# hmakelin/gisnav

Measured on AMD Instinct MI355X. Metric: matched frame-pairs/sec + PnP poses/sec, 640x480 cam-vs-tile, higher is better.
Workload: dtype f32-accurate FFN / out-projection / match-head GEMMs (each f32 operand split into 2 fp16 terms = 22 significant bits, 3 fp16 MFMA partial products, f32 accumulate; fp16-range guard active); attention INPUT projections (q, k, v: 18 of 66 launches) on 2 partial products -- the fp16 high term of the ac

## Files before the change

### gisnav_amd/csrc/gn_api.hip

```cpp
#include "gn_common.h"

#include <cstdio>
#include <cstring>
#include <cmath>
#include <cctype>
#include <algorithm>
#include <tuple>

using namespace gn;

namespace {

thread_local std::string g_err;

struct Linear { float* w = nullptr; float* b = nullptr; int out = 0, in = 0; uint16_t* wp = nullptr; float acc_scale = 1.f;
                uint16_t* wf = nullptr; int frag_order = -1;
                uint16_t* wf2 = nullptr;
                uint16_t* wfn = nullptr; };

struct Block {
  Linear proj_in;
  Linear proj_out;
  Linear ffn0;
  float* ln_g = nullptr; float* ln_b = nullptr;
// ... 3 lines not shown

enum Stage { ST_PREP = 0, ST_PROJ, ST_ATTN, ST_FFN, ST_HEAD, ST_GATHER, ST_PNP, ST_COUNT };

struct Call {
  int B = 0, kpt_format = 0, stride_q = 0, stride_r = 0;
  const float *desc_q = nullptr, *kpt_q = nullptr, *desc_r = nullptr, *kpt_r = nullptr; const int32_t *n_q = nullptr, *n_r = nullptr;
  const uint8_t* dem = nullptr; int H = 0, W = 0;
  double *R = nullptr, *t = nullptr; int32_t *n_match = nullptr, *n_inliers = nullptr; uint8_t* ok = nullptr; int64_t* idx = nullptr; float* score = nullptr;
  double *cov = nullptr, *sigma_hat = nullptr; uint8_t* cov_ok = nullptr; double sigma_px = 0.0;
  const double* K9 = nullptr; int min_matches = 0;
  int kw = 0, in_dim = 0; size_t km = 0;
  Call() = default;
  Call(int feature, int npad, int B_, int kpt_format_, const float* desc_q_, const float* kpt_q_, const int32_t* n_q_, int stride_q_,
       const float* desc_r_, const float* kpt_r_, const int32_t* n_r_, int stride_r_)
      : B(B_), kpt_format(kpt_format_), stride_q(stride_q_), stride_r(stride_r_), desc_q(desc_q_), kpt_q(kpt_q_), desc_r(desc_r_), kpt_r(kpt_r_),
        n_q(n_q_), n_r(n_r_), kw((kpt_format_ & 0xff) == GN_KPT_LAF ? 6 : (kpt_format_ & 0xff) == GN_KPT_RECORD ? kRecordFloats : 4),
        in_dim(feature == GN_FEATURE_SIFT ? kInDim : kDim), km((size_t)npad) {}
};

template <typename F, typename... C> void pair_arrays(const Call& h, F&& f, C&... c) {
  f((size_t)h.stride_q * h.in_dim * 4, false, c.desc_q...); f((size_t)h.stride_r * h.in_dim * 4, false, c.desc_r...);
  f((size_t)h.stride_q * h.kw * 4, false, c.kpt_q...); f((size_t)h.stride_r * h.kw * 4, false, c.kpt_r...);
  f((size_t)4, false, c.n_q...); f((size_t)4, false, c.n_r...); f((size_t)h.H * h.W, false, c.dem...);
  f((size_t)72, true, c.R...); f((size_t)24, true, c.t...); f((size_t)4, true, c.n_match...); f((size_t)4, true, c.n_inliers...); f((size_t)1, true, c.ok...);
  f(h.km * 16, true, c.idx...); f(h.km * 4, true, c.score...);
  f((size_t)288, true, c.cov...); f((size_t)8, true, c.sigma_hat...); f((size_t)1, true, c.cov_ok...);
}
template <typename T> T* byte_offset(T* p, size_t bytes) { return reinterpret_cast<T*>(reinterpret_cast<uintptr_t>(p) + bytes); }

Call slice(const Call& v, size_t b0, int n) {
  Call o = v;
  o.B = n;
  pair_arrays(o, [&](size_t bytes, bool, auto*& p) { if (p) p = byte_offset(p, b0 * bytes); }, o);
  return o;
}

template <typename... T> struct Restore {
  std::tuple<T&...> ref; std::tuple<T...> val;
  explicit Restore(T&... r) : ref(r...), val(r...) {}
  ~Restore() { ref = val; }
  Restore(const Restore&) = delete;
  Restore& operator=(const Restore&) = delete;
};

}

struct gn_ctx {
  int device = 0, max_batch = 0, npad = 0, precision = 0;
  int x_planes_only = 1;
  int qkv_stamps = 0;
  int qkv_fused = 1;
  int sp_split = 1;
  long long sp_split_trips = 0;
  int sp_stop = 0;
  int sp_ts_layer = 0;
  long long* sp_ts = nullptr;
  void* sp_allocs_dbg = nullptr;
  bool sp_enc_hm16 = false, sp_enc_fp16 = false;
  int head_fused = 1;
  int head_stamps = 0;
  int pnp_stamps = 0;
  int ffn_compose = 1;
  int ffn_fold = 1;
  int ffn_fused = 3;
  unsigned int* ovf_base = nullptr; unsigned int* ovf = nullptr; unsigned int* ovf_host = nullptr;
  int dbg_trip_group = 0;
  bool in_group = false;
  int ovf_groups_last = 1;
  int guard = 1;
  long long guard_trips = 0;
  int certify = 0;
  float cert_eps = 4.0e-3f;
  int cert_eps_src = 0;
  float cert_eps_f32 = 1.0e-4f;
  float* max0b = nullptr; float* rpart_c = nullptr; int32_t* uncert = nullptr; int32_t* uncert_alt = nullptr; int32_t* uncert_host = nullptr;
  bool cert_inner = false;
  void* cert_stage = nullptr; size_t cert_stage_bytes = 0;
  struct CertPending {
    bool active = false; hipEvent_t ev = nullptr; int32_t* flags = nullptr;
    int npad_run = 0, level = 0;
    Call call; double K9[9] = {0};
  } cert_pend[2];
  int cert_slot = 0;
  long long cert_calls = 0, cert_pairs = 0, cert_flag_margin = 0, cert_flag_range = 0, cert_rerun = 0, cert_f32_marginal = 0;
  int attn_f16 = 0;
  int ladder = 0; float cert_eps_mid = -1.f, cert_mid_measured = -1.f;
  long long mid_rerun = 0, mid_certified = 0, mid_passed = 0;
  float *colbest = nullptr, *col2 = nullptr;
  bool cal_cols = false;
  int precision_api = 0;
  int feature = 0;
  float size_q[2] = {0.f, 0.f}, size_r[2] = {0.f, 0.f};
  int npad_run = 0;
  int n_layers = kMaxLayers;
  float threshold = 0.5f;
  std::string err;
  Linear input_proj;
  float* wr = nullptr;
  Block self_blk[kMaxLayers], cross_blk[kMaxLayers];
  Linear final_proj[kMaxLayers], matchability[kMaxLayers];
  std::map<std::string, bool> loaded;
  std::vector<std::string> required;
  float *desc = nullptr, *cos_t = nullptr, *sin_t = nullptr, *extent = nullptr;
  int32_t* nvalid = nullptr;
  float *x = nullptr, *qkv = nullptr, *ctx = nullptr, *msg = nullptr, *h = nullptr, *md = nullptr, *ls = nullptr;
  uint16_t *desc_p = nullptr, *x_p = nullptr, *ctx_p = nullptr, *msg_p = nullptr, *h_p = nullptr, *md_p = nullptr;
  size_t Tmax = 0;
  int planes_mode = 0;
  float* sim = nullptr;
  uint16_t *qkb = nullptr, *vtb = nullptr;
  float* attn_part = nullptr; unsigned int* attn_tickets = nullptr;
  int attn_split = 1;
  int attn_variant = 4;
  int stop_after = 0;
  int launch_count = 0;
  int no_planes = 0;
  int dbg_planes = 0;
  uint16_t* dbg_wp = nullptr; size_t dbg_wp_n = 0;
  int dbg_out = 0;
  uint16_t* dbg_yp = nullptr; size_t dbg_yp_n = 0;
  int dbg_vt_skip = 0;
  int dbg_reuse = 0;
  uint16_t* dbg_ap = nullptr; size_t dbg_ap_n = 0;
  int gemm_variant = -1;
  float *rowmax = nullptr, *rowlog = nullptr, *colmax = nullptr, *collog = nullptr, *max0 = nullptr;
  int32_t *m0 = nullptr, *m1 = nullptr;
  float *cpart_m = nullptr, *cpart_s = nullptr;
  int32_t* cpart_i = nullptr;
  float* rot4 = nullptr;
  float *rpart_a = nullptr, *rpart_b = nullptr;
  unsigned int* tickets = nullptr;
  int64_t* e_idx = nullptr; float* e_score = nullptr; float* e_mkp = nullptr; float* e_obj = nullptr;
  int defer_join = 0, sub_last_B = 0, sub_last_np = 0;
  int sub_serial = 0;
  int cu_mask_mode = 0;
  int use_lists = 1;
  int ncu = 256;
  int fused_proj_status = -1;
  bool fused_proj_pending = true;
  int fused_proj_off = 0;
  int qkv_in_tail = 1;
  int skinny = 1;
  int auto_level = 3; float cert_eps_lvl[2] = {-1.f, -1.f}; long long auto_pairs = 0, auto_wide = 0, auto_narrow = 0, auto_calls_lvl[2] = {0, 0}, auto_switches = 0;
  int ffn_products = 3;
  int qkv_products = 2;
  unsigned long long* tile_feedback = nullptr;
  int* lists = nullptr; long long lists_stride = 0;
  int n_sub = 1; hipStream_t sub_s[8] = {}; hipEvent_t ev_fork = nullptr; hipEvent_t ev_join[8] = {}; bool sub_pending[8] = {};
  int overlap = 0; unsigned long long calls = 0;
  hipStream_t s_pnp = nullptr; hipEvent_t ev_gather[2][8] = {}, ev_pnp[2][8] = {}; bool pnp_pending[2][8] = {}, pnp_recorded[2][8] = {};
  hipEvent_t ev_head[8] = {};
  float* o_mkp[2] = {nullptr, nullptr}; float* o_obj[2] = {nullptr, nullptr}; int32_t* o_nmatch[2] = {nullptr, nullptr};
  int prep_fused = 1;
  int sift_h = 0, sift_w = 0; std::vector<void*> sift_allocs; SiftPyramid sift_py; float* sift_tmp = nullptr;
  float* sift_dk = nullptr; std::vector<std::vector<float>> sift_kernels; std::vector<int> sift_koff;
  int4* sift_cand = nullptr; int* sift_counts = nullptr; SiftKeypoint* sift_kp = nullptr;
  int sift_max_cand = 0, sift_max_kp = 0, sift_raw_cap = 0, sift_batch = 0; long long sift_kp_stride = 0;
  std::vector<int32_t> sift_totals;
  struct SpConv { float* wf = nullptr; float* b = nullptr; int cout = 0, cin = 0, taps = 0, cout_pad = 0; bool have_w = false, have_b = false;
                  uint16_t* wfh = nullptr; float acc_scale = 1.f; };
  SpConv sp[12];
  std::vector<void*> sp_allocs; int sp_h = 0, sp_w = 0, sp_chunk = 0, sp_cap = 0, sp_max = 0;
  float *sp_x = nullptr, *sp_y = nullptr, *sp_z = nullptr, *sp_maps[6] = {};
  int *sp_cand = nullptr, *sp_counts = nullptr, *sp_index = nullptr;
  float* vo_norm2 = nullptr; int32_t* vo_nn_idx = nullptr; float* vo_nn_dist = nullptr; uint8_t* vo_good = nullptr;
  uint8_t* mask_ws = nullptr;
  float* pts_ws = nullptr;
  gn::HypResult* hyp_ws = nullptr;
  std::vector<void*> allocs;
  std::vector<void*> ws_allocs;
  bool timing = false;
  hipEvent_t ev[2 * 128];
  int ev_stage[128]; int n_ev = 0; bool ev_ready = false;
  float stage_ms[ST_COUNT] = {0};
  bool ktiming = false;
  std::vector<hipEvent_t> kev;
  std::vector<double> kflops;
  std::vector<double> kbytes;
  std::vector<int> kclass;
  std::vector<const char*> kname;
  size_t kused = 0;
};

namespace {

#define GN_HIP(call)                                                                              \
  do {                                                                                            \
    hipError_t e_ = (call);                                                                       \
    if (e_ != hipSuccess) {                                                                       \
      char buf_[512];                                                                             \
      snprintf(buf_, sizeof buf_, "%s failed: %s (%s:%d)", #call, hipGetErrorString(e_), __FILE__, __LINE__); \
      if (ctx) ctx->err = buf_;                                                                   \
      g_err = buf_;                                                                               \
      return GN_ERR_HIP;                                                                          \
    }                                                                                             \
  } while (0)

int fail(gn_ctx* ctx, int code, const std::string& msg) {
  if (ctx) ctx->err = msg;
  g_err = msg;
  return code;
}

template <typename T>
int dalloc(gn_ctx* ctx, T** p, size_t count) {
  void* q = nullptr;
  GN_HIP(hipMalloc(&q, count * sizeof(T)));
  GN_HIP(hipMemset(q, 0, count * sizeof(T)));
  ctx->allocs.push_back(q);
  *p = reinterpret_cast<T*>(q);
  return GN_OK;
}

template <typename T_>
int ws_alloc(gn_ctx* ctx, T_** p, size_t count) {
  void* q = nullptr;
  GN_HIP(hipMalloc(&q, count * sizeof(T_)));
  GN_HIP(hipMemset(q, 0, count * sizeof(T_)));
  ctx->ws_allocs.push_back(q);
  *p = reinterpret_cast<T_*>(q);
  return GN_OK;
}
int ensure_sim(gn_ctx* ctx) {
  if (ctx->sim) return GN_OK;
  return ws_alloc(ctx, &ctx->sim, (size_t)ctx->max_batch * ctx->npad * ctx->npad);
}

std::string canonical(const std::string& k) {
  for (const char* kind : {"self_attn.", "cross_attn."}) {
    const size_t L = strlen(kind);
    if (k.compare(0, L, kind) == 0) {
      const size_t dot = k.find('.', L);
      if (dot == std::string::npos) return k;
      return "transformers." + k.substr(L, dot - L) + "." + std::string(kind) + k.substr(dot + 1);
    }
  }
  return k;
}

struct StageTimer {
  gn_ctx* c; hipStream_t s; int st;
  StageTimer(gn_ctx* c_, hipStream_t s_, int st_) : c(c_), s(s_), st(st_) {
    if (c->timing && c->n_ev < 128) { hipEventRecord(c->ev[2 * c->n_ev], s); }
  }
  ~StageTimer() {
    if (c->timing && c->n_ev < 128) { hipEventRecord(c->ev[2 * c->n_ev + 1], s); c->ev_stage[c->n_ev] = st; ++c->n_ev; }
  }
};

bool planes_of(gn_ctx* c, const float* p, uint16_t** planes) {
  struct { const float* f; uint16_t* q; size_t cols; } tab[] = {
    {c->desc, c->desc_p, (size_t)kInDim}, {c->x, c->x_p, (size_t)kDim}, {c->ctx, c->ctx_p, (size_t)kDim},
    {c->msg, c->msg_p, (size_t)kDim}, {c->h, c->h_p, (size_t)2 * kDim}, {c->md, c->md_p, (size_t)kDim}};
  for (auto& e : tab) {
    if (e.f && p >= e.f && p < e.f + c->Tmax * e.cols && (size_t)(p - e.f) % e.cols == 0) {
      *planes = e.q + 2 * (p - e.f);
      return true;
    }
  }
  return false;
}

template <typename F> bool timed_launch(gn_ctx* c, hipStream_t s, int kclass, double flops, double bytes, const char* name, F&& launch) {
  ++c->launch_count;
  if (c->stop_after && c->launch_count > c->stop_after) return false;
  const bool rec = c->ktiming && c->kused < c->kflops.size();
  if (rec) hipEventRecord(c->kev[2 * c->kused], s);
  launch();
  if (rec) {
    hipEventRecord(c->kev[2 * c->kused + 1], s);
    c->kflops[c->kused] = flops; c->kbytes[c->kused] = bytes; c->kclass[c->kused] = kclass; c->kname[c->kused] = name ? name : gn::g_last_kernel;
    ++c->kused;
  }
  return true;
}

void timed_gemm(gn_ctx* c, int epi, const GemmArgs& g_in, int batch, hipStream_t s) {
  if (c->gemm_variant >= 0) gn::g_gemm_variant = c->gemm_variant;
  GemmArgs g = g_in;
  if (c->no_planes) g.Wp = nullptr;
  bool p2 = false;
  if (c->planes_mode) {
    uint16_t* q = nullptr;
    p2 = planes_of(c, g.A, &q);
    if (p2) {
      g.Ap = q;
      if (g.A2) { uint16_t* q2 = nullptr; p2 = planes_of(c, g.A2, &q2) && g.lda2 == g.lda; g.A2p = q2; }
    }
    if (p2 && !g.Wp) {
      uint16_t* qw = nullptr;
      p2 = planes_of(c, g.W, &qw);
      g.Wp = qw; g.acc_scale = 1.f;
    }
    if (p2) g.ovf = c->guard ? c->ovf : nullptr;
    if (p2) {
      uint16_t* qy = nullptr;
      if (g.Y == c->x) { planes_of(c, g.Y, &qy); g.Yp = qy; g.ldyp = g.ldy; if (g.drop_f32) g.Y = nullptr; }
      else if (g.Y == c->msg || g.Y == c->md) { planes_of(c, g.Y, &qy); g.Yp = qy; g.ldyp = g.ldy; g.Y = nullptr; }
      else if (epi == EPI_LN_GELU && g.Y == c->h) { planes_of(c, g.Y, &qy); g.Yp = qy; g.ldyp = g.ldy; g.Y = nullptr; }
    }
  }
  const double mn = (double)g.M * g.N * batch;
  double by = 4.0 * ((double)g.M * g.K * batch + (double)g.N * g.K * (g.strideW ? batch : 1));
  if (epi == EPI_ROTARY_BF16 || epi == EPI_SCALE_BF16) by += 2.0 * mn;
  else if (epi == EPI_LN_GELU) by += 4.0 * mn;
  else if (epi != EPI_LN_GELU) by += (g.Y ? 4.0 * mn : 0.0) + (g.Yp ? 4.0 * mn : 0.0);
  if (epi == EPI_RESIDUAL) by += 4.0 * mn;
  if (epi == EPI_ROTARY || epi == EPI_ROTARY_BF16) by += 2.0 * 4.0 * (double)g.M * kFreq;
  timed_launch(c, s, 0, 2.0 * g.M * (double)g.N * g.K * batch, by, nullptr, [&] { if (p2) launch_gemm_p2(epi, g, batch, s); else launch_gemm_f32(epi, g, batch, s); });
}

void gemm(gn_ctx* c, int epi, GemmArgs& g, hipStream_t s) {
  g.strideA = g.strideW = g.strideY = 0;
  timed_gemm(c, epi, g, 1, s);
}

int build_planes(gn_ctx* ctx, Linear& L) {
  if (!L.w || L.out <= 0 || L.in <= 0) return GN_OK;
  const size_t n = (size_t)L.out * L.in;
  if (!L.wp) { int rc = dalloc(ctx, &L.wp, 3 * n); if (rc != GN_OK) return rc; }
  if (ctx->precision == GN_PREC_F16X2_BF16_ATTN) {
    std::vector<float> host(n);
    GN_HIP(hipMemcpy(host.data(), L.w, n * sizeof(float), hipMemcpyDeviceToHost));
    float mx = 0.f;
    for (float v : host) { const float av = fabsf(v); if (av > mx) mx = av; }
    int e = 0;
    if (mx > 0.f && std::isfinite(mx)) { frexpf(mx, &e); e = 13 - e; }
    if (e > 60) e = 60;
    if (e < -60) e = -60;
    const float scale = ldexpf(1.0f, e);
    L.acc_scale = ldexpf(1.0f, -e);
    if (ctx->planes_mode) launch_split_hm16(L.w, L.wp, L.out, L.in, scale, 0);
    else launch_split2_f16(L.w, L.wp, (long long)n, scale, 0);
    if (ctx->planes_mode && L.frag_order >= 0 && L.out % 32 == 0 && L.in % 16 == 0) {
      std::vector<uint16_t> frag(2 * n);
      build_weight_fragments(host.data(), L.out, L.in, scale, L.frag_order, frag.data());
      if (!L.wf) { int rc = dalloc(ctx, &L.wf, 2 * n); if (rc != GN_OK) return rc; }
      GN_HIP(hipMemcpy(L.wf, frag.data(), frag.size() * sizeof(uint16_t), hipMemcpyHostToDevice));
      if (L.frag_order == 1) {
        build_weight_fragments(host.data(), L.out, L.in, scale, 0, frag.data());
        if (!L.wfn) { int rc = dalloc(ctx, &L.wfn, 2 * n); if (rc != GN_OK) return rc; }
        GN_HIP(hipMemcpy(L.wfn, frag.data(), frag.size() * sizeof(uint16_t), hipMemcpyHostToDevice));
      }
      if (L.out == 2 * kDim && L.in == 2 * kDim) {
        build_weight_fragments(host.data(), L.out, L.in, scale, 2, frag.data());
        if (!L.wf2) { int rc = dalloc(ctx, &L.wf2, 2 * n); if (rc != GN_OK) return rc; }
        GN_HIP(hipMemcpy(L.wf2, frag.data(), frag.size() * sizeof(uint16_t), hipMemcpyHostToDevice));
      }
    }
  } else {
    L.acc_scale = 1.f;
    launch_split3_bf16(L.w, L.wp, (long long)n, 0);
  }
  GN_HIP(hipStreamSynchronize(0));
  return GN_OK;
}

GemmArgs gemm_args(const float* A, int lda, const Linear& L, float* Y, int ldy, int M) {
  GemmArgs g;
  memset(&g, 0, sizeof g);
  g.Wp = L.wp; g.wp_plane = (long long)L.out * L.in; g.acc_scale = L.acc_scale;
  g.A = A; g.lda = lda; g.A2 = nullptr; g.lda2 = 0; g.K1 = L.in;
  g.W = L.w; g.ldw = L.in; g.bias = L.b; g.Y = Y; g.ldy = ldy; g.M = M; g.N = L.out; g.K = L.in;
  return g;
}

static void attn_split(gn_ctx* c, AttnArgs& a) {
  const int blocks = a.npad / 128 * kHeads * a.BS;
  int S = 1;
  while (S < 4 && S < c->attn_split && blocks * S * 2 <= (c->attn_split >= 8 ? 512 : 256) && a.npad / 64 >= 4 * S) S *= 2;
  if (c->attn_part && c->attn_tickets && c->attn_split && c->n_sub <= 1 && S > 1) { a.nsplit = S; a.part = c->attn_part; a.tickets = c->attn_tickets; }
}

void attention(gn_ctx* c, const AttnArgs& a, hipStream_t s) {
  if (c->precision != GN_PREC_F32 && c->attn_f16 == 2) launch_attention_f16x2(a, s);
  else if (c->precision != GN_PREC_F32) launch_attention_bf16(a, s); else launch_attention_f32(a, s);
}

void timed_attention(gn_ctx* c, const AttnArgs& a, bool bf16v2, hipStream_t s) {
  timed_launch(c, s, 1, 4.0 * a.BS * kHeads * (double)a.npad * a.npad * kHeadDim,
               (double)a.BS * a.npad * kDim * (a.qb ? 2.0 + 2.0 + 2.0 : 12.0) + (double)a.BS * a.npad * kDim * 4.0,
               nullptr, [&] { if (bf16v2) launch_attention_bf16_v2(a, s); else attention(c, a, s); });
}

bool qkv_projection_applies(const gn_ctx* c, const Block& blk, int T, int np, int vt_perm) {
  return c->planes_mode && c->qkv_fused && blk.proj_in.wf && c->x_p && c->qkb && c->vtb && c->rot4 && T % 128 == 0 && np % 128 == 0 && (vt_perm & 1) &&
         (T / 128 >= 128 || c->qkv_fused == 2);
}
bool skinny_applies(const gn_ctx* c, int T, int np) {
  return (c->skinny & 3) && c->planes_mode && c->x_planes_only && T % 32 == 0 && np > 0 && ((c->skinny & 3) == 2 || T / np <= 4);
}
bool qkv_projection(gn_ctx* c, const Block& blk, bool cross, int T, int np, int vt_perm, hipStream_t s) {
  const bool skinny = skinny_applies(c, T, np) && !(c->skinny & 4) && c->qkv_fused && blk.proj_in.wf && c->x_p && c->qkb && c->vtb && c->rot4 && np % 32 == 0 && vt_perm == 1 && !c->qkv_stamps;
  if (!skinny && !qkv_projection_applies(c, blk, T, np, vt_perm)) return false;
  QkvArgs q;
  q.xp = c->x_p; q.wf = blk.proj_in.wf; q.acc_scale = blk.proj_in.acc_scale; q.bias = blk.proj_in.b;
  q.rot4 = c->rot4; q.rot_stride = (long long)c->Tmax; q.qkb = c->qkb; q.ldyb = cross ? kDim : 2 * kDim; q.vt = c->vtb; q.npad = np;
  q.qscale = 0.125f; q.scale = 0.35355339059327373f; q.vt_perm = vt_perm; q.T = T;
  q.half_fmt = c->attn_f16; q.ovf = (c->attn_f16 && c->guard) ? c->ovf : nullptr;
  q.tiles = (c->use_lists && c->lists && !c->qkv_stamps) ? c->lists : nullptr;
  q.products = c->qkv_products == 3 ? 3 : 2; q.ncu = c->ncu;
  q.dbg_ts = (c->qkv_stamps && c->sim) ? reinterpret_cast<long long*>(c->sim) : nullptr;
  const double N = cross ? 2.0 * kDim : 3.0 * kDim;
  timed_launch(c, s, 0, 2.0 * T * N * kDim, 4.0 * T * kDim + 2.0 * T * N + 4.0 * N * kDim + (cross ? 0.0 : 2.0 * 4.0 * T * kFreq),
               nullptr, [&] { if (skinny) launch_skinny_qkv(q, cross, s); else launch_qkv(q, cross, s); });
  return true;
}

int build_composed(gn_ctx* ctx, Block& blk) {
  if (!blk.comp_dirty) return GN_OK;
  const Linear &F = blk.ffn0, &P = blk.proj_out;
  if (!ctx->planes_mode || !F.w || !F.b || !P.w || !P.b || F.out != 2 * kDim || F.in != 2 * kDim || P.out != kDim || P.in != kDim) return GN_OK;
  const int H = 2 * kDim, D = kDim;
  std::vector<float> w1((size_t)H * H), b1(H), wo((size_t)D * D), bo(D);
  GN_HIP(hipMemcpy(w1.data(), F.w, w1.size() * 4, hipMemcpyDeviceToHost));
  GN_HIP(hipMemcpy(b1.data(), F.b, b1.size() * 4, hipMemcpyDeviceToHost));
  GN_HIP(hipMemcpy(wo.data(), P.w, wo.size() * 4, hipMemcpyDeviceToHost));
  GN_HIP(hipMemcpy(bo.data(), P.b, bo.size() * 4, hipMemcpyDeviceToHost));
  std::vector<float> wc((size_t)H * H), bc(H);
  std::vector<double> row(D);
  float mx = 0.f;
  for (int h = 0; h < H; ++h) {
    const float* w1h = &w1[(size_t)h * H];
    for (int k = 0; k < D; ++k) { row[k] = 0.0; wc[(size_t)h * H + k] = w1h[k]; }
    double bb = b1[h];
    for (int f = 0; f < D; ++f) {
      const double wm = w1h[D + f];
      const float* wof = &wo[(size_t)f * D];
      for (int k = 0; k < D; ++k) row[k] += wm * wof[k];
      bb += wm * bo[f];
    }
    for (int k = 0; k < D; ++k) wc[(size_t)h * H + D + k] = (float)row[k];
    bc[h] = (float)bb;
    for (int k = 0; k < H; ++k) { const float av = fabsf(wc[(size_t)h * H + k]); if (av > mx) mx = av; }
  }
  int e = 0;
  if (mx > 0.f && std::isfinite(mx)) { frexpf(mx, &e); e = 13 - e; }
  if (e > 60) e = 60;
  if (e < -60) e = -60;
  std::vector<uint16_t> frag((size_t)2 * H * H);
  build_weight_fragments(wc.data(), H, H, ldexpf(1.0f, e), 0, frag.data());
  if (!blk.wfc) { int rc = dalloc(ctx, &blk.wfc, frag.size()); if (rc != GN_OK) return rc; }
  if (!blk.b1c) { int rc = dalloc(ctx, &blk.b1c, (size_t)H); if (rc != GN_OK) return rc; }
  GN_HIP(hipMemcpy(blk.wfc, frag.data(), frag.size() * sizeof(uint16_t), hipMemcpyHostToDevice));
  GN_HIP(hipMemcpy(blk.b1c, bc.data(), bc.size() * sizeof(float), hipMemcpyHostToDevice));
  blk.wfc_scale = ldexpf(1.0f, -e);
  blk.comp_dirty = false;
  return GN_OK;
}

int ensure_composed(gn_ctx* ctx) {
  if (!ctx->planes_mode || !ctx->ffn_compose) return GN_OK;
  for (int i = 0; i < ctx->n_layers; ++i) {
    int rc = build_composed(ctx, ctx->self_blk[i]); if (rc != GN_OK) return rc;
    rc = build_composed(ctx, ctx->cross_blk[i]); if (rc != GN_OK) return rc;
  }
  return GN_OK;
}

bool tail_folds_out_proj(const gn_ctx* c, const Block& blk, int T) {
  return c->planes_mode && c->x_planes_only && c->ffn_fused == 3 && c->ffn_fold && blk.ffn0.wf && blk.ffn0.wf2 && blk.ffn3.wf && blk.proj_out.wf &&
         T % 64 == 0 && c->precision != GN_PREC_F32 && c->attn_variant >= 1;
}

bool tail_should_walk(const gn_ctx* c) {
  if (!c->tile_feedback) return false;
  const int g = (int)(c->ovf - c->ovf_base);
  if (g < 0 || g >= 8) return false;
  const unsigned long long w = __atomic_load_n(&c->tile_feedback[g], __ATOMIC_RELAXED);
  const unsigned all = (unsigned)(w >> 32), valid = (unsigned)w;
  return all > 0 && (unsigned long long)valid * 10u < (unsigned long long)all * 9u;
}

inline bool ffn_auto(const gn_ctx* c) { return c->ffn_products == 0 && c->cert_eps_lvl[0] >= 0.f && c->cert_eps_lvl[1] >= 0.f && c->certify >= 2; }
inline int ffn_level(const gn_ctx* c) { return c->attn_f16 == 2 ? 3 : c->ffn_products == 0 ? (ffn_auto(c) ? c->auto_level : 3) : c->ffn_products; }
inline float cert_eps_now(const gn_ctx* c) { return ffn_auto(c) ? c->cert_eps_lvl[c->auto_level - 2] : c->cert_eps; }

bool ffn(gn_ctx* c, const Block& blk, int T, hipStream_t s, bool keep_f32, const Block* next = nullptr, bool next_cross = false, int np = 0, int vt_perm = 0) {
  if (skinny_applies(c, T, np) && !(c->skinny & 8) && c->ffn_fused == 3 && c->ffn_compose && tail_folds_out_proj(c, blk, T) && blk.wfc && blk.b1c && !blk.comp_dirty && blk.ffn3.wfn &&
      c->h && c->ctx_p && gn::g_ffn_stamps == 0 && gn::g_ffn_shape == 0) {
    SkinnyTailArgs a;
    a.xp = c->x_p; a.cp = c->ctx_p; a.w1 = blk.wfc; a.w1_scale = blk.wfc_scale; a.b1 = blk.b1c; a.h = c->h; a.ln_g = blk.ln_g; a.ln_b = blk.ln_b;
    a.w2 = blk.ffn3.wfn; a.w2_scale = blk.ffn3.acc_scale; a.b2 = blk.ffn3.b; a.xp_out = c->x_p; a.y = keep_f32 ? c->x : nullptr;
    a.ovf = c->guard ? c->ovf : nullptr; a.T = T;
    if (!timed_launch(c, s, 0, 2.0 * T * 512.0 * 512.0, 4.0 * T * (256.0 + 256.0 + 512.0) + 4.0 * 512.0 * 512.0, nullptr, [&] { launch_skinny_h(a, s, c->skinny >> 4); })) return false;
    timed_launch(c, s, 0, 2.0 * T * 256.0 * 512.0, 4.0 * T * (512.0 + 256.0 + 256.0) + 4.0 * 256.0 * 512.0, nullptr, [&] { launch_skinny_out(a, s, c->skinny >> 4); });
    return false;
  }
  if (c->planes_mode && c->x_planes_only && c->ffn_fused == 3 && blk.ffn0.wf && blk.ffn3.wf && T % 64 == 0) {
    FfnArgs f;
    const bool fold = tail_folds_out_proj(c, blk, T);
    f.cp = fold ? c->ctx_p : nullptr; f.wos = blk.proj_out.wf; f.wo_scale = blk.proj_out.acc_scale; f.bo = blk.proj_out.b;
    f.xp = c->x_p; f.mp = c->msg_p; f.w1s = fold ? blk.ffn0.wf2 : blk.ffn0.wf; f.w1_scale = blk.ffn0.acc_scale; f.b1 = blk.ffn0.b; f.ln_g = blk.ln_g; f.ln_b = blk.ln_b;
    f.w2s = blk.ffn3.wf; f.w2_scale = blk.ffn3.acc_scale; f.b2 = blk.ffn3.b; f.yp = c->x_p; f.y = keep_f32 ? c->x : nullptr; f.T = T;
    const bool comp = fold && c->ffn_compose && blk.wfc && blk.b1c && !blk.comp_dirty;
    if (comp) { f.composed = 1; f.w1s = blk.wfc; f.w1_scale = blk.wfc_scale; f.b1 = blk.b1c; }
    f.ovf = c->guard ? c->ovf : nullptr;
    f.tiles = (c->use_lists && c->lists && gn::g_ffn_stamps == 0) ? c->lists : nullptr;
    f.walk = c->use_lists == 2 || (c->use_lists == 1 && tail_should_walk(c));
    f.ncu = c->ncu;
    f.composed = comp ? 1 : 0;
    f.products = (comp && ffn_level(c) == 2) ? 2 : 3;
    const bool fuse_qkv = next != nullptr && c->qkv_in_tail && !c->fused_proj_off && comp && ffn_selects_128(f) && gn::g_ffn_stamps == 0 && c->attn_f16 && c->qkv_products != 3 && !c->qkv_stamps &&
                          c->precision != GN_PREC_F32 && c->attn_variant >= 1 && qkv_projection_applies(c, *next, T, np, vt_perm) && !(vt_perm & 2);
    if (fuse_qkv) {
      f.qkv = next_cross ? 2 : 1;
      f.q_wf = next->proj_in.wf; f.q_acc_scale = next->proj_in.acc_scale; f.q_bias = next->proj_in.b;
      f.q_rot4 = c->rot4; f.q_rot_stride = (long long)c->Tmax; f.q_qkb = c->qkb; f.q_vt = c->vtb;
      f.q_qscale = 0.125f; f.q_scale = 0.35355339059327373f;
      f.npad = np;
    }
    if (c->use_lists) { f.nvalid = c->nvalid; f.npad = c->npad_run; }
    f.dbg_ts = gn::g_ffn_stamps ? reinterpret_cast<long long*>(c->sim) : nullptr;
    double flops = 2.0 * T * (512.0 * 512.0 + 256.0 * 512.0 + ((fold && !comp) ? 256.0 * 256.0 : 0.0));
    double bytes = 4.0 * T * (256.0 + 256.0 + 256.0 + 256.0) + 4.0 * (512.0 * 512.0 + 256.0 * 512.0);
    if (fuse_qkv) {
      const double N = next_cross ? 2.0 * kDim : 3.0 * kDim;
      flops += 2.0 * T * N * kDim;
      bytes += 2.0 * T * N + 4.0 * N * kDim + (next_cross ? 0.0 : 2.0 * 4.0 * T * kFreq);
    }
    return timed_launch(c, s, 0, flops, bytes, nullptr, [&] { launch_ffn_fused(f, s); }) && fuse_qkv;
  }
  GemmArgs g = gemm_args(c->x, kDim, blk.ffn0, c->h, 2 * kDim, T);
  g.A2 = c->msg; g.lda2 = kDim; g.K1 = kDim;
  if (c->planes_mode && T % 128 == 0 && (c->ffn_fused == 2 || (c->ffn_fused == 1 && T / 128 >= 256))) {
    g.ln_g = blk.ln_g; g.ln_b = blk.ln_b;
    gemm(c, EPI_LN_GELU, g, s);
  } else {
    gemm(c, EPI_BIAS, g, s);
    launch_ln_gelu(c->h, blk.ln_g, blk.ln_b, T, s, c->planes_mode ? c->h_p : nullptr, c->planes_mode && c->guard ? c->ovf : nullptr);
  }
  GemmArgs g3 = gemm_args(c->h, 2 * kDim, blk.ffn3, c->x, kDim, T);
  g3.resid = c->x; g3.ldr = kDim;
  if (c->planes_mode && c->x_planes_only) {
    uint16_t* xp = nullptr;
    if (planes_of(c, c->x, &xp)) { g3.residp = xp; g3.ldrp = kDim; g3.resid = nullptr; g3.drop_f32 = keep_f32 ? 0 : 1; }
  }
  gemm(c, EPI_RESIDUAL, g3, s);
  return false;
}

int run_matcher(gn_ctx* c, const Call& v, hipStream_t s) {
  const int B = v.B, np = c->npad_run, T = B * 2 * np, BS = B * 2;
  const bool bf16v2 = c->precision != GN_PREC_F32 && c->attn_variant >= 1 && c->attn_f16 != 2;
  gn::g_attn_variant = c->attn_variant;
  gn::g_attn_stamps = (c->attn_variant == 73 && c->sim) ? reinterpret_cast<long long*>(c->sim) : nullptr;
  const int vt_perm = (bf16v2 ? 1 : 0) | (c->dbg_vt_skip ? 2 : 0);
  const bool attn_planes = c->planes_mode && (bf16v2 || c->attn_f16 == 2);
  c->launch_count = 0;
  {
    StageTimer tm(c, s, ST_PREP);
    PrepArgs p;
    p.desc_q = v.desc_q; p.kpt_q = v.kpt_q; p.n_q = v.n_q; p.stride_q = v.stride_q;
    p.desc_r = v.desc_r; p.kpt_r = v.kpt_r; p.n_r = v.n_r; p.stride_r = v.stride_r;
    p.kpt_format = v.kpt_format; p.B = B; p.npad = np; p.wr = c->wr;
    p.desc = c->desc; p.kxy = nullptr; p.cos_t = c->cos_t; p.sin_t = c->sin_t; p.nvalid = c->nvalid; p.extent = c->extent;
    p.size_q[0] = c->size_q[0]; p.size_q[1] = c->size_q[1]; p.size_r[0] = c->size_r[0]; p.size_r[1] = c->size_r[1];
    p.feature = c->feature; p.x = nullptr; p.xp = nullptr;
    p.ovf_clear = (c->planes_mode && c->guard) ? c->ovf : nullptr;
    p.ovf_init = (c->dbg_trip_group && c->ovf == c->ovf_base + (c->dbg_trip_group - 1)) ? 1u : 0u;
    p.desc_p = nullptr; p.rot4 = nullptr; p.rot_stride = (long long)c->Tmax;
    const bool planes_only = c->planes_mode && c->x_planes_only && c->n_layers > 0;
    if (c->feature == 1) {
      p.x = planes_only ? nullptr : c->x; p.xp = c->planes_mode ? c->x_p : nullptr;
      launch_prep(p, s);
      if (c->rot4 && c->qkv_fused) launch_rot_table(c->cos_t, c->sin_t, c->rot4, T, (long long)c->Tmax, s);
    } else {
      const bool rot = c->rot4 && c->qkv_fused, split = c->planes_mode != 0;
      if (c->prep_fused) { p.rot4 = rot ? c->rot4 : nullptr; p.desc_p = split ? c->desc_p : nullptr; }
      launch_prep(p, s);
      if (rot && !p.rot4) launch_rot_table(c->cos_t, c->sin_t, c->rot4, T, (long long)c->Tmax, s);
      if (split && !p.desc_p) launch_split_hm16(c->desc, c->desc_p, T, kInDim, 1.0f, s);
      GemmArgs g = gemm_args(c->desc, kInDim, c->input_proj, c->x, kDim, T);
      g.drop_f32 = planes_only ? 1 : 0;
      gemm(c, EPI_BIAS, g, s);
    }
  }
  if (c->use_lists && c->lists) {
    const int g = (int)(c->ovf - c->ovf_base);
    launch_tile_lists(c->nvalid, BS, np, c->lists, (c->tile_feedback && g >= 0 && g < 8) ? c->tile_feedback + g : nullptr, s);
  }
  bool qkv_done = false;
  for (int i = 0; i < c->n_layers; ++i) {
    {
      const Block& blk = c->self_blk[i];
      if (!qkv_done) {
        StageTimer tm(c, s, ST_PROJ);
        GemmArgs g = gemm_args(c->x, kDim, blk.proj_in, c->qkv, 3 * kDim, T);
        g.cos_t = c->cos_t; g.sin_t = c->sin_t; g.rot_cols = 2 * kDim;
        if (bf16v2 && qkv_projection(c, blk, false, T, np, vt_perm, s)) {
        } else if (bf16v2) {
          g.Yb = c->qkb; g.ldyb = 2 * kDim; g.Vt = c->vtb; g.vt_start = 2 * kDim; g.q_cols = kDim; g.qscale = 0.125f; g.npad = np; g.vt_perm = vt_perm; g.half_fmt = c->attn_f16;
          gemm(c, EPI_ROTARY_BF16, g, s);
        } else {
          gemm(c, EPI_ROTARY, g, s);
        }
      }
      {
        StageTimer tm(c, s, ST_ATTN);
        AttnArgs a; a.ovf = nullptr;
        a.q = c->qkv; a.ldq = 3 * kDim; a.k = c->qkv + kDim; a.ldk = 3 * kDim; a.v = c->qkv + 2 * kDim; a.ldv = 3 * kDim;
        a.out = c->ctx; a.ldo = kDim; a.nvalid = c->nvalid; a.npad = np; a.cross = 0; a.qscale = 0.125f; a.BS = BS;
        a.outp = attn_planes ? c->ctx_p : nullptr; a.ovf = (attn_planes && c->guard) ? c->ovf : nullptr;
        a.qb = c->qkb; a.ldqb = 2 * kDim; a.kb = c->qkb + kDim; a.ldkb = 2 * kDim; a.vt = c->vtb; a.half_fmt = c->attn_f16; a.tiles = (c->use_lists && c->lists) ? c->lists : nullptr; a.ncu = c->ncu;
        if (bf16v2) attn_split(c, a);
        timed_attention(c, a, bf16v2, s);
        if (c->planes_mode && !attn_planes) launch_split_hm16(c->ctx, c->ctx_p, T, kDim, 1.0f, s);
      }
      if (!tail_folds_out_proj(c, blk, T)) {
        StageTimer tm(c, s, ST_PROJ);
        GemmArgs g = gemm_args(c->ctx, kDim, blk.proj_out, c->msg, kDim, T);
        gemm(c, EPI_BIAS, g, s);
      }
      { StageTimer tm(c, s, ST_FFN); qkv_done = ffn(c, blk, T, s, false, bf16v2 ? &c->cross_blk[i] : nullptr, true, np, vt_perm); }
    }
    {
      const Block& blk = c->cross_blk[i];
      if (!qkv_done) {
        StageTimer tm(c, s, ST_PROJ);
        GemmArgs g = gemm_args(c->x, kDim, blk.proj_in, c->qkv, 2 * kDim, T);
        g.scale = 0.35355339059327373f;
        g.scale_cols = kDim;
        if (bf16v2 && qkv_projection(c, blk, true, T, np, vt_perm, s)) {
        } else if (bf16v2) {
          g.Yb = c->qkb; g.ldyb = kDim; g.Vt = c->vtb; g.vt_start = kDim; g.q_cols = 0; g.qscale = 1.0f; g.npad = np; g.vt_perm = vt_perm; g.half_fmt = c->attn_f16;
          gemm(c, EPI_SCALE_BF16, g, s);
        } else {
          gemm(c, EPI_SCALE_COLS, g, s);
        }
      }
      {
        StageTimer tm(c, s, ST_ATTN);
        AttnArgs a; a.ovf = nullptr;
        a.q = c->qkv; a.ldq = 2 * kDim; a.k = c->qkv; a.ldk = 2 * kDim; a.v = c->qkv + kDim; a.ldv = 2 * kDim;
        a.out = c->ctx; a.ldo = kDim; a.nvalid = c->nvalid; a.npad = np; a.cross = 1; a.qscale = 1.0f; a.BS = BS;
        a.outp = attn_planes ? c->ctx_p : nullptr; a.ovf = (attn_planes && c->guard) ? c->ovf : nullptr;
        a.qb = c->qkb; a.ldqb = kDim; a.kb = c->qkb; a.ldkb = kDim; a.vt = c->vtb; a.half_fmt = c->attn_f16; a.tiles = (c->use_lists && c->lists) ? c->lists : nullptr; a.ncu = c->ncu;
        if (bf16v2) attn_split(c, a);
        timed_attention(c, a, bf16v2, s);
        if (c->planes_mode && !attn_planes) launch_split_hm16(c->ctx, c->ctx_p, T, kDim, 1.0f, s);
      }
      if (!tail_folds_out_proj(c, blk, T)) {
        StageTimer tm(c, s, ST_PROJ);
        GemmArgs g = gemm_args(c->ctx, kDim, blk.proj_out, c->msg, kDim, T);
        gemm(c, EPI_BIAS, g, s);
      }
      { StageTimer tm(c, s, ST_FFN); qkv_done = ffn(c, blk, T, s, i == c->n_layers - 1, (bf16v2 && i + 1 < c->n_layers) ? &c->self_blk[i + 1] : nullptr, false, np, vt_perm); }
    }
  }
  {
    StageTimer tm(c, s, ST_HEAD);
    const int li = c->n_layers - 1;
    GemmArgs g = gemm_args(c->x, kDim, c->final_proj[li], c->md, kDim, T);
    g.scale = 0.25f; g.scale_cols = kDim;
    gemm(c, EPI_SCALE_COLS, g, s);
    launch_matchability(c->x, c->matchability[li].w, c->matchability[li].b, c->ls, T, s);
    HeadArgs hd;
    hd.sim = c->sim; hd.ls = c->ls; hd.nvalid = c->nvalid; hd.B = B; hd.npad = np; hd.threshold = c->threshold;
    hd.rowmax = c->rowmax; hd.rowlog = c->rowlog; hd.colmax = c->colmax; hd.collog = c->collog;
    hd.m0 = c->m0; hd.max0 = c->max0; hd.m1 = c->m1;
    hd.ovf = (c->planes_mode && c->guard) ? c->ovf : nullptr;
    hd.max0b = c->max0b; hd.rpart_c = c->rpart_c; hd.uncert = c->certify ? c->uncert : nullptr;
    hd.cert_eps = (c->precision == GN_PREC_F32) ? c->cert_eps_f32 : cert_eps_now(c);
    if (hd.uncert && c->precision != GN_PREC_F32 && ffn_auto(c)) { hd.uncert_alt = c->uncert_alt; hd.cert_eps_alt = c->cert_eps_lvl[3 - c->auto_level]; }
    hd.idx = v.idx; hd.score = v.score; hd.n_match = v.n_match; hd.kmax = c->npad;
    hd.md = c->planes_mode ? (const void*)c->md_p : (const void*)c->md; hd.md_f32 = c->planes_mode ? 0 : 1;
    hd.cpart_m = c->cpart_m; hd.cpart_s = c->cpart_s; hd.cpart_i = c->cpart_i; hd.rpart_a = c->rpart_a; hd.rpart_b = c->rpart_b; hd.tickets = c->tickets;
    hd.dbg_ts = (c->head_stamps && c->sim) ? reinterpret_cast<long long*>(c->sim) : nullptr;
    if (c->cal_cols) { hd.colbest = c->colbest; hd.col2 = c->col2; }
    if (c->head_fused || !c->sim) {
      timed_launch(c, s, 0, 2.0 * 2.0 * B * (double)np * np * kDim,
                   2.0 * (4.0 * T * kDim) + 4.0 * T * 4.0 + 8.0 * B * np * 3.0,
                   "k_head_fused (2 sweeps)", [&] { launch_match_head_fused(hd, s); });
      return GN_OK;
    }
    GemmArgs gs;
    memset(&gs, 0, sizeof gs);
    gs.A = c->md; gs.lda = kDim; gs.K1 = kDim; gs.W = c->md + (size_t)np * kDim; gs.ldw = kDim;
    gs.Y = c->sim; gs.ldy = np; gs.M = np; gs.N = np; gs.K = kDim; gs.acc_scale = 1.f;
    gs.strideA = gs.strideW = 2LL * np * kDim; gs.strideY = (long long)np * np;
    timed_gemm(c, EPI_PLAIN, gs, B, s);
    launch_match_head(hd, s);
  }
  return GN_OK;
}

int alloc_workspace(gn_ctx* ctx, int max_kpts) {
  ctx->npad = ((max_kpts + 127) / 128) * 128;
  ctx->npad_run = ctx->npad;
  const size_t np = ctx->npad, T = (size_t)ctx->max_batch * 2 * np, B = ctx->max_batch;
#define GN_ALLOC(field, count)                                     \
  do { int rc_ = ws_alloc(ctx, &ctx->field, (count)); if (rc_ != GN_OK) return rc_; } while (0)
  GN_ALLOC(desc, T * kInDim); GN_ALLOC(cos_t, T * kFreq); GN_ALLOC(sin_t, T * kFreq);
  GN_ALLOC(extent, B * 4); GN_ALLOC(nvalid, B * 2);
  GN_ALLOC(x, T * kDim); GN_ALLOC(qkv, T * 3 * kDim); GN_ALLOC(ctx, T * kDim); GN_ALLOC(msg, T * kDim);
  GN_ALLOC(h, T * 2 * kDim); GN_ALLOC(md, T * kDim); GN_ALLOC(ls, T);
  ctx->Tmax = T;
  if (ctx->precision == GN_PREC_F16X2_BF16_ATTN) {
    ctx->planes_mode = 1;
    GN_ALLOC(desc_p, 2 * T * kInDim); GN_ALLOC(x_p, 2 * T * kDim); GN_ALLOC(ctx_p, 2 * T * kDim);
    GN_ALLOC(msg_p, 2 * T * kDim); GN_ALLOC(h_p, 2 * T * 2 * kDim); GN_ALLOC(md_p, 2 * T * kDim);
    GN_ALLOC(rot4, T * 2 * kFreq);
  }
  if (ctx->precision != GN_PREC_F32) { GN_ALLOC(qkb, T * 2 * kDim); GN_ALLOC(vtb, T * kDim); GN_ALLOC(attn_part, (size_t)256 * 4 * 34 * 64); GN_ALLOC(attn_tickets, 256); }
  GN_ALLOC(rowmax, B * np); GN_ALLOC(rowlog, B * np); GN_ALLOC(colmax, B * np); GN_ALLOC(collog, B * np);
  GN_ALLOC(max0, B * np); GN_ALLOC(m0, B * np); GN_ALLOC(m1, B * np); GN_ALLOC(max0b, B * np); GN_ALLOC(rpart_c, B * 8 * np); GN_ALLOC(uncert, B); GN_ALLOC(uncert_alt, B);
  GN_ALLOC(colbest, B * np); GN_ALLOC(col2, B * np);
  GN_ALLOC(cpart_m, B * (np / 32) * np); GN_ALLOC(cpart_s, B * (np / 32) * np); GN_ALLOC(cpart_i, B * (np / 32) * np); GN_ALLOC(rpart_a, B * 8 * np); GN_ALLOC(rpart_b, B * 8 * np); GN_ALLOC(tickets, B * 2);
  GN_ALLOC(e_idx, B * np * 2); GN_ALLOC(e_score, B * np); GN_ALLOC(e_mkp, B * np * 2); GN_ALLOC(e_obj, B * np * 3);
  GN_ALLOC(vo_norm2, T); GN_ALLOC(vo_nn_idx, B * np * 2); GN_ALLOC(vo_nn_dist, B * np * 2); GN_ALLOC(vo_good, B * np);
  GN_ALLOC(mask_ws, B * np * 16);
  GN_ALLOC(pts_ws, B * np * 5);
  GN_ALLOC(hyp_ws, B * 16);
  GN_ALLOC(ovf_base, 16);
  ctx->ovf = ctx->ovf_base;
  ctx->lists_stride = gn::kTileListBase + 2 * (np / 128) + 8 * ((np + 255) / 256);
  GN_ALLOC(lists, B * (size_t)ctx->lists_stride);
#undef GN_ALLOC
  return GN_OK;
}

void shift_workspaces(gn_ctx* c, long long b0, int sign);

__global__ void k_count_diff(const uint4* a, const uint4* b, size_t n, unsigned int* cnt) {
  bool d = false;
  for (size_t i = (size_t)blockIdx.x * blockDim.x + threadIdx.x; i < n; i += (size_t)gridDim.x * blockDim.x) {
    const uint4 x = a[i], y = b[i];
    d |= (x.x != y.x) | (x.y != y.y) | (x.z != y.z) | (x.w != y.w);
  }
  const unsigned long long bal = __ballot(d);
  if ((threadIdx.x & 63) == 0 && bal) atomicAdd(cnt, (unsigned int)__popcll(bal));
}

int selfcheck_fused_projection(gn_ctx* c) {
  gn_ctx* ctx = c;
  c->fused_proj_pending = false;
  c->fused_proj_status = -1;
  c->fused_proj_off = 0;
  const int np = c->npad;
  GN_HIP(hipDeviceSynchronize());
  if (!c->planes_mode || !c->qkv_in_tail || !c->attn_f16 || c->attn_f16 == 2 || c->qkv_products == 3 || !c->ffn_compose || c->ffn_fused != 3 || !c->x_planes_only || c->n_layers < 1 ||
      !c->qkv_fused || !c->rot4 || !c->lists || !c->msg_p || !c->h_p || c->feature < 0 || gn::g_ffn_stamps != 0 || gn::g_ffn_shape != 0) return GN_OK;
  int B = (256 * 128 + 2 * np - 1) / (2 * np);
  if (B > c->max_batch) return GN_OK;
  const int T = B * 2 * np;
  std::vector<float> h((size_t)T * kDim);
  unsigned long long st = 0x9E3779B97F4A7C15ull;
  auto rnd = [&]() { st ^= st << 13; st ^= st >> 7; st ^= st << 17; return (float)((st >> 40) & 0xFFFF) * (1.0f / 32768.0f) - 1.0f; };
  for (int pass = 0; pass < 2; ++pass) {
    for (auto& v : h) v = 1.5f * rnd();
    float* dst = pass == 0 ? c->x : c->ctx;
    GN_HIP(hipMemcpy(dst, h.data(), h.size() * sizeof(float), hipMemcpyHostToDevice));
    launch_split_hm16(dst, pass == 0 ? c->x_p : c->ctx_p, T, kDim, 1.0f, 0);
  }
  {
    std::vector<float> cs((size_t)T * kFreq), sn((size_t)T * kFreq);
    for (size_t i = 0; i < cs.size(); ++i) { const float th = 3.14159265f * rnd(); cs[i] = cosf(th); sn[i] = sinf(th); }
    GN_HIP(hipMemcpy(c->cos_t, cs.data(), cs.size() * sizeof(float), hipMemcpyHostToDevice));
    GN_HIP(hipMemcpy(c->sin_t, sn.data(), sn.size() * sizeof(float), hipMemcpyHostToDevice));
    launch_rot_table(c->cos_t, c->sin_t, c->rot4, T, (long long)c->Tmax, 0);
    std::vector<int32_t> nv(2 * (size_t)B, np);
    GN_HIP(hipMemcpy(c->nvalid, nv.data(), nv.size() * sizeof(int32_t), hipMemcpyHostToDevice));
    launch_tile_lists(c->nvalid, 2 * B, np, c->lists, nullptr, 0);
  }
  const size_t xbytes = (size_t)T * kDim * 4, qbytes = (size_t)T * 2 * kDim * 2, vbytes = (size_t)T * kDim * 2;
  uint16_t* const keep_q = c->h_p;
  uint16_t* const keep_v = c->h_p + (size_t)T * 2 * kDim;
  GN_HIP(hipMemcpy(c->msg_p, c->x_p, xbytes, hipMemcpyDeviceToDevice));
  unsigned int* cnt = c->ovf_base + 12;
  GN_HIP(hipMemset(cnt, 0, sizeof(unsigned int)));
  bool applicable = true;
  {
    const Restore keep(c->use_lists, c->qkv_in_tail, c->guard, c->ktiming, c->launch_count, c->stop_after, c->npad_run, c->ffn_products);
    const int prod0 = c->ffn_products;
    c->ktiming = false; c->stop_after = 0; c->guard = 0; c->npad_run = np;
    const int nblk = c->n_layers > 1 ? 1 : 0;
    const int n_lv = (prod0 == 0 || prod0 == 2) ? 2 : 1;
    for (int lv = 0; lv < n_lv && applicable; ++lv)
    for (int cross = 0; cross < 2 && applicable; ++cross)
      for (int walk = 0; walk < 2 && applicable; ++walk) {
        c->ffn_products = lv == 0 ? 3 : 2;
        const Block& tail = cross ? c->self_blk[0] : c->cross_blk[0];
        const Block* next = cross ? &c->cross_blk[0] : &c->self_blk[nblk];
        c->use_lists = walk ? 2 : 3;
        GN_HIP(hipMemcpyAsync(c->x_p, c->msg_p, xbytes, hipMemcpyDeviceToDevice, 0));
        GN_HIP(hipMemsetAsync(c->qkb, 0, qbytes, 0)); GN_HIP(hipMemsetAsync(c->vtb, 0, vbytes, 0));
        c->qkv_in_tail = 1;
        if (!ffn(c, tail, T, 0, false, next, cross != 0, np, 1)) { applicable = false; break; }
        GN_HIP(hipMemcpyAsync(keep_q, c->qkb, qbytes, hipMemcpyDeviceToDevice, 0));
        GN_HIP(hipMemcpyAsync(keep_v, c->vtb, vbytes, hipMemcpyDeviceToDevice, 0));
        GN_HIP(hipMemcpyAsync(c->x_p, c->msg_p, xbytes, hipMemcpyDeviceToDevice, 0));
        GN_HIP(hipMemsetAsync(c->qkb, 0, qbytes, 0)); GN_HIP(hipMemsetAsync(c->vtb, 0, vbytes, 0));
        c->qkv_in_tail = 0;
        ffn(c, tail, T, 0, false, next, cross != 0, np, 1);
        if (!qkv_projection(c, *next, cross != 0, T, np, 1, 0)) { applicable = false; break; }
        hipLaunchKernelGGL(k_count_diff, dim3(1024), dim3(256), 0, 0, reinterpret_cast<const uint4*>(keep_q), reinterpret_cast<const uint4*>(c->qkb), (cross ? qbytes / 2 : qbytes) / 16, cnt);
        hipLaunchKernelGGL(k_count_diff, dim3(1024), dim3(256), 0, 0, reinterpret_cast<const uint4*>(keep_v), reinterpret_cast<const uint4*>(c->vtb), vbytes / 16, cnt);
      }
  }
  unsigned int diffs = 0;
  GN_HIP(hipStreamSynchronize(0));
  GN_HIP(hipMemcpy(&diffs, cnt, sizeof diffs, hipMemcpyDeviceToHost));
  GN_HIP(hipMemset(c->x_p, 0, xbytes)); GN_HIP(hipMemset(c->ctx_p, 0, xbytes)); GN_HIP(hipMemset(c->msg_p, 0, xbytes)); GN_HIP(hipMemset(c->h_p, 0, qbytes + vbytes));
  GN_HIP(hipMemset(c->qkb, 0, qbytes)); GN_HIP(hipMemset(c->vtb, 0, vbytes)); GN_HIP(hipMemset(c->x, 0, xbytes)); GN_HIP(hipMemset(c->ctx, 0, xbytes));
  GN_HIP(hipMemset(cnt, 0, sizeof(unsigned int)));
  if (!applicable) return GN_OK;
  c->fused_proj_status = diffs == 0 ? 1 : 0;
  if (diffs != 0) {
    c->fused_proj_off = 1;
    fprintf(stderr, "[gisnav_amd] the projection fused behind the block tail differs from the separate k_qkv launches in %u 16-byte words on this context's weights: "
                    "fusion switched off for this context (results stay correct, ~4 %% slower)\n", diffs);
  }
  return GN_OK;
}

void ffn_level_update(gn_ctx* c, int B, const int32_t* flags, const int32_t* alt, int lvl) {
  if (!ffn_auto(c) || c->precision == GN_PREC_F32 || lvl < 2 || lvl > 3) return;
  ++c->auto_calls_lvl[lvl - 2];
  int nf = 0, na = 0;
  for (int b = 0; b < B; ++b) { nf += flags[b] == 1; na += alt[b] == 1; }
  c->auto_pairs += B; c->auto_wide += lvl == 2 ? nf : na; c->auto_narrow += lvl == 2 ? na : nf;
  if (c->auto_pairs < 64) return;
  const int next = (c->auto_wide - c->auto_narrow) * 64 <= c->auto_pairs ? 2 : 3;
  if (next != c->auto_level) ++c->auto_switches;
  c->auto_level = next;
  c->auto_pairs = c->auto_wide = c->auto_narrow = 0;
}

struct ExactF32 : Restore<int, int, int, int, int> {
  explicit ExactF32(gn_ctx* c) : Restore(c->precision, c->planes_mode, c->gemm_variant, c->no_planes, c->attn_f16) {
    c->precision = GN_PREC_F32; c->planes_mode = 0; c->gemm_variant = 3; c->no_planes = 1; c->attn_f16 = 0;
  }
};
struct MidLevel : Restore<int, int, int, float> {
  explicit MidLevel(gn_ctx* c) : Restore(c->attn_f16, c->ffn_products, c->dbg_trip_group, c->cert_eps) {
    c->attn_f16 = 2; c->ffn_products = 3; c->dbg_trip_group = 0; c->cert_eps = c->cert_eps_mid;
  }
};
struct F32x3 : Restore<int, int, int, int> {
  explicit F32x3(gn_ctx* c) : Restore(c->planes_mode, c->gemm_variant, c->no_planes, c->attn_f16) {
    c->planes_mode = 0; c->gemm_variant = 5; c->no_planes = 1; c->attn_f16 = 0;
  }
};
inline bool ladder_active(const gn_ctx* c) { return c->ladder && c->cert_eps_mid >= 0.f && c->precision != GN_PREC_F32 && c->planes_mode && c->attn_f16 != 2; }

template <typename F> int rerun_pairs(gn_ctx* ctx, hipStream_t s, const Call& v, F& run, const std::vector<int>& flagged, std::vector<int32_t>& rflags) {
  const int nf = (int)flagged.size();
  const bool contiguous = flagged.back() - flagged.front() + 1 == nf;
  int rc = GN_OK;
  Call st = slice(v, 0, nf);
  if (!contiguous) {
    auto place = [&](char* base) {
      size_t off = 0;
      pair_arrays(st, [&](size_t bytes, bool, auto*& p) {
        if (!p) return;
        if (base) p = reinterpret_cast<std::remove_reference_t<decltype(p)>>(base + off);
        off = (off + nf * bytes + 255) & ~(size_t)255;
      }, st);
      return off;
    };
    const size_t need = place(nullptr);
    if (need > ctx->cert_stage_bytes) {
      if (ctx->cert_stage) { GN_HIP(hipStreamSynchronize(s)); GN_HIP(hipFree(ctx->cert_stage)); ctx->cert_stage = nullptr; ctx->cert_stage_bytes = 0; }
      GN_HIP(hipMalloc(&ctx->cert_stage, need));
      ctx->cert_stage_bytes = need;
    }
    place(static_cast<char*>(ctx->cert_stage));
  }
  auto copy_pair = [&](const Call& dst, size_t bd, const Call& src, size_t bs, bool outputs) {
    hipError_t e = hipSuccess;
    pair_arrays(v, [&](size_t bytes, bool out, auto* d, auto* q) {
      if (d && out == outputs && e == hipSuccess)
        e = hipMemcpyAsync(const_cast<void*>(static_cast<const void*>(byte_offset(d, bd * bytes))), byte_offset(q, bs * bytes), bytes, hipMemcpyDeviceToDevice, s);
    }, dst, src);
    return e;
  };
  if (!contiguous)
    for (int k = 0; k < nf; ++k) GN_HIP(copy_pair(st, k, v, flagged[k], false));
  {
    const Restore keep(ctx->cert_inner, ctx->in_group, ctx->ovf);
    ctx->cert_inner = true; ctx->in_group = true; ctx->ovf = ctx->ovf_base;
    if (contiguous) {
      const int b0 = flagged.front();
      shift_workspaces(ctx, b0, +1);
      rc = run(slice(v, b0, nf));
      shift_workspaces(ctx, b0, -1);
    } else {
      rc = run(st);
    }
  }
  if (rc != GN_OK) return rc;
  if (!contiguous)
    for (int k = 0; k < nf; ++k) GN_HIP(copy_pair(v, flagged[k], st, k, true));
  GN_HIP(hipMemcpyAsync(ctx->uncert_host, ctx->uncert, (size_t)v.B * sizeof(int32_t), hipMemcpyDeviceToHost, s));
  GN_HIP(hipStreamSynchronize(s));
  rflags.resize(nf);
  for (int k = 0; k < nf; ++k) rflags[k] = ctx->uncert_host[contiguous ? flagged[k] : k];
  return GN_OK;
}

template <typename F> int certify_rerun(gn_ctx* ctx, hipStream_t s, const Call& v, F&& run, const int32_t* flags_ready = nullptr, int flags_level = 0) {
  const int B = v.B;
  if (!flags_ready) {
    GN_HIP(hipMemcpyAsync(ctx->uncert_host, ctx->uncert, (size_t)B * sizeof(int32_t), hipMemcpyDeviceToHost, s));
    if (ffn_auto(ctx)) GN_HIP(hipMemcpyAsync(ctx->uncert_host + ctx->max_batch, ctx->uncert_alt, (size_t)B * sizeof(int32_t), hipMemcpyDeviceToHost, s));
    GN_HIP(hipStreamSynchronize(s));
    flags_ready = ctx->uncert_host;
  }
  ffn_level_update(ctx, B, flags_ready, flags_ready + ctx->max_batch, flags_level ? flags_level : ctx->auto_level);
  ++ctx->cert_calls; ctx->cert_pairs += B;
  std::vector<int> flagged, margin;
  for (int b = 0; b < B; ++b) {
    const int f = flags_ready[b];
    if (f == 1) ++ctx->cert_flag_margin; else if (f == 2) ++ctx->cert_flag_range;
    if (f != 0) flagged.push_back(b);
    if (f == 1) margin.push_back(b);
  }
  if (flagged.empty()) return GN_OK;
  if (ctx->precision == GN_PREC_F32) { ctx->cert_f32_marginal += (long long)flagged.size(); return GN_OK; }
  std::vector<int32_t> rflags;
  if (ladder_active(ctx) && !margin.empty()) {
    std::vector<int> still(flagged.size() - margin.size());
    std::copy_if(flagged.begin(), flagged.end(), still.begin(), [&](int b) { return flags_ready[b] != 1; });
    int rc = GN_OK;
    { const MidLevel mid(ctx); rc = rerun_pairs(ctx, s, v, run, margin, rflags); }
    if (rc != GN_OK) return rc;
    ctx->mid_rerun += (long long)margin.size();
    for (size_t k = 0; k < margin.size(); ++k) {
      if (rflags[k] == 0) ++ctx->mid_certified;
      else { ++ctx->mid_passed; still.push_back(margin[k]); }
    }
    std::sort(still.begin(), still.end());
    flagged.swap(still);
    if (flagged.empty()) return GN_OK;
  }
  int rc = GN_OK;
  { const ExactF32 f32(ctx); rc = rerun_pairs(ctx, s, v, run, flagged, rflags); }
  ctx->cert_rerun += (long long)flagged.size();
  if (rc != GN_OK) return rc;
  for (int32_t f : rflags) if (f != 0) ++ctx->cert_f32_marginal;
  return GN_OK;
}

enum { kCalExactF32 = 0, kCalMid = 1 };
struct CalPass { std::vector<float> best, second, colbest, col2; unsigned int trip = 0u; };
int cal_pass(gn_ctx* ctx, const Call& w, int arith, bool cols, std::vector<int32_t>* nv, CalPass& out, hipStream_t s) {
  int rc = GN_OK;
// ... 1266 lines not shown
    memcpy(host_out, &trips, 8);
    return 1;
  }
  if (strcmp(name, "e_idx") == 0) {
    size_t count = B * np * 2;
    if ((int64_t)(count * 8) > max_bytes) count = (size_t)max_bytes / 8;
    if (hipStreamSynchronize((hipStream_t)stream) != hipSuccess) return GN_ERR_HIP;
    if (hipMemcpy(host_out, ctx->e_idx, count * 8, hipMemcpyDeviceToHost) != hipSuccess) return GN_ERR_HIP;
    return (int64_t)count;
  }
  return fail(ctx, GN_ERR_NAME, std::string("unknown debug tensor ") + name);
}

int gn_debug_gemm(gn_ctx* ctx, int M, int N, int K, const float* A, const float* W, const float* bias, float* Y, void* stream) {
  if (!ctx || !A || !W || !Y || M % 128 || N % 128 || K % 32 || M < 128 || N < 128 || K < 32)
    return fail(ctx, GN_ERR_ARG, "gn_debug_gemm needs M,N multiples of 128 and K a multiple of 32");
  GN_HIP(hipSetDevice(ctx->device));
  GemmArgs g;
  memset(&g, 0, sizeof g);
  g.A = A; g.lda = K; g.K1 = K; g.W = W; g.ldw = K; g.bias = bias; g.Y = Y; g.ldy = N; g.M = M; g.N = N; g.K = K;
  g.acc_scale = 1.f;
  if (ctx->gemm_variant >= 0) gn::g_gemm_variant = ctx->gemm_variant;
  if (ctx->gemm_variant == 7) {
    
    const size_t na = (size_t)M * K, nw = (size_t)N * K;
    if (ctx->dbg_ap_n < na) { ctx->dbg_ap = nullptr; int rc = dalloc(ctx, &ctx->dbg_ap, 2 * na); if (rc != GN_OK) return rc; ctx->dbg_ap_n = na; }
    if (ctx->dbg_wp_n < nw) { ctx->dbg_wp = nullptr; int rc = dalloc(ctx, &ctx->dbg_wp, 3 * nw); if (rc != GN_OK) return rc; ctx->dbg_wp_n = nw; }
    const int e = ctx->dbg_planes > 0 ? ctx->dbg_planes - 1 : 0;
    if (!ctx->dbg_reuse) {
      launch_split_hm16(A, ctx->dbg_ap, M, K, 1.0f, (hipStream_t)stream);
      launch_split_hm16(W, ctx->dbg_wp, N, K, ldexpf(1.0f, e), (hipStream_t)stream);
    }
    g.Ap = ctx->dbg_ap; g.Wp = ctx->dbg_wp; g.acc_scale = ldexpf(1.0f, -e);
    if (ctx->dbg_out) {
      const size_t ny = (size_t)M * N;
      if (ctx->dbg_yp_n < ny) { ctx->dbg_yp = nullptr; int rc = dalloc(ctx, &ctx->dbg_yp, 2 * ny); if (rc != GN_OK) return rc; ctx->dbg_yp_n = ny; }
      g.Yp = ctx->dbg_yp; g.ldyp = N;
      if (ctx->dbg_out == 1) g.Y = nullptr;
    }
    launch_gemm_p2(bias ? EPI_BIAS : EPI_PLAIN, g, 1, (hipStream_t)stream);
    GN_HIP(hipGetLastError());
    return GN_OK;
  }
  if (ctx->dbg_planes) {
    const size_t n = (size_t)N * K;
    if (ctx->dbg_wp_n < n) { ctx->dbg_wp = nullptr; int rc = dalloc(ctx, &ctx->dbg_wp, 3 * n); if (rc != GN_OK) return rc; ctx->dbg_wp_n = n; }
    if (ctx->gemm_variant == 6 || ctx->gemm_variant >= 60) {
      launch_split2_f16(W, ctx->dbg_wp, (long long)n, ldexpf(1.0f, ctx->dbg_planes - 1), (hipStream_t)stream);
      g.acc_scale = ldexpf(1.0f, 1 - ctx->dbg_planes);
    } else {
      launch_split3_bf16(W, ctx->dbg_wp, (long long)n, (hipStream_t)stream);
    }
    g.Wp = ctx->dbg_wp; g.wp_plane = (long long)n;
  }
  launch_gemm_f32(bias ? EPI_BIAS : EPI_PLAIN, g, 1, (hipStream_t)stream);
  GN_HIP(hipGetLastError());
  return GN_OK;
}

int gn_debug_attention(gn_ctx* ctx, int BS, int npad, int cross, float qscale, const float* q, int ldq, const float* k, int ldk,
                       const float* v, int ldv, const int32_t* nkv, float* out, int ldo, void* stream) {
  if (!ctx || !q || !k || !v || !nkv || !out || npad % 128 || BS < 1 || (cross && (BS & 1)))
    return fail(ctx, GN_ERR_ARG, "bad gn_debug_attention argument");
  GN_HIP(hipSetDevice(ctx->device));
  AttnArgs a; a.ovf = nullptr;
  a.q = q; a.ldq = ldq; a.k = k; a.ldk = ldk; a.v = v; a.ldv = ldv; a.out = out; a.ldo = ldo;
  a.nvalid = nkv; a.npad = npad; a.cross = cross; a.qscale = qscale; a.BS = BS;
  a.qb = a.kb = a.vt = nullptr; a.ldqb = a.ldkb = 0; a.outp = nullptr; a.half_fmt = ctx->attn_f16; a.ncu = ctx->ncu;
  const long long cap = (long long)ctx->max_batch * 2 * ctx->npad;
  if (ctx->precision != GN_PREC_F32 && ctx->attn_f16 != 2 && ctx->attn_variant >= 1 && ctx->qkb && ctx->vtb && (long long)BS * npad <= cap) {
    launch_pack_attn_bf16(a, ctx->qkb, ctx->vtb, (hipStream_t)stream);
    a.qb = ctx->qkb; a.kb = ctx->qkb + kDim; a.ldqb = a.ldkb = 2 * kDim; a.vt = ctx->vtb;
    gn::g_attn_variant = ctx->attn_variant;
    gn::g_attn_stamps = (ctx->attn_variant == 73 && ctx->sim) ? reinterpret_cast<long long*>(ctx->sim) : nullptr;
    attn_split(ctx, a);
    launch_attention_bf16_v2(a, (hipStream_t)stream);
  } else {
    attention(ctx, a, (hipStream_t)stream);
  }
  GN_HIP(hipGetLastError());
  return GN_OK;
}

int gn_sp_set_arithmetic(gn_ctx* ctx, int mode) {
  if (!ctx || mode < GN_SP_EXACT_F32 || mode > GN_SP_FP16) return GN_ERR_ARG;
  if (mode != GN_SP_EXACT_F32 && ctx->precision != GN_PREC_F16X2_BF16_ATTN) return fail(ctx, GN_ERR_ARG, "the fp16 SuperPoint arithmetic needs a context of the f16x2 precision");
  ctx->sp_split = mode;
  return GN_OK;
}

static bool retired_variant(int which, int value) {
  switch (which) {
    case 0: return (value >= 51 && value <= 57) || (value >= 61 && value <= 67);
    case 1: return (value >= 41 && value <= 46) || value == 48 || (value >= 51 && value <= 55) || value == 57 || value == 58 ||
                   value == 71 || value == 72 || value >= 1000;
    case 8: return value != 0 && value != 1;
    case 12: return value != 0 && value != 8 && value != 136;
    default: return false;
  }
}

int gn_debug_set_variant(gn_ctx* ctx, int which, int value) {
  if (!ctx || retired_variant(which, value)) return GN_ERR_ARG;
  if ((which == 1 && value == 73) || (which == 12 && (value & 8)) || (which == 15 && value) || (which == 16 && !value) || (which == 17 && value) || (which == 20 && value)) {
    GN_HIP(hipSetDevice(ctx->device));
    const int rc = ensure_sim(ctx); if (rc != GN_OK) return rc;
  }
  if (which == 0) { gn::g_gemm_variant = value; ctx->gemm_variant = value; }
  else if (which == 1) ctx->attn_variant = value;
  else if (which == 2) ctx->dbg_planes = value;
  else if (which == 3) ctx->no_planes = value;
  else if (which == 4) ctx->stop_after = value;
  else if (which == 5) ctx->planes_mode = (value && ctx->x_p) ? 1 : 0;
  else if (which == 6) ctx->dbg_reuse = value;
  else if (which == 7) ctx->dbg_out = value;
  else if (which == 10) ctx->ffn_fused = value;
  else if (which == 11) ctx->x_planes_only = value;
  else if (which == 8) gn::g_p2_wide = value;
  else if (which == 9) ctx->dbg_vt_skip = value;
  else if (which == 12) gn::g_ffn_stamps = value;
  else if (which == 13) ctx->ffn_fold = value;
  else if (which == 14) gn::g_ffn_shape = value;
  else if (which == 15) ctx->pnp_stamps = value;
  else if (which == 16) ctx->head_fused = value;
  else if (which == 17) ctx->head_stamps = value;
  else if (which == 19) ctx->qkv_fused = value;
  else if (which == 20) ctx->qkv_stamps = value;
  else if (which == 21) ctx->sp_split = value;
  else if (which == 24) gn::g_sp_conv_h = value;
  else if (which == 34) gn::g_sp_conv_s = value;
  else if (which == 36) gn::g_sp_nms_fused = value;
  else if (which == 40) gn::g_sp_select_stream = value;
  else if (which == 41) gn::g_gemm_m64 = value;
  else if (which == 42) gn::g_lf_conv_knob = value;
  else if (which == 43) gn::g_attn_f32_ks = value;
  else if (which == 44) gn::g_gemm_r64 = value;
  else if (which == 46) gn::g_sp_fuse1 = value;
  else if (which == 47) { ctx->fused_proj_pending = value == 0; }
  else if (which == 39) ctx->sp_stop = value;
  else if (which == 35) {
    ctx->sp_ts_layer = value;
    if (value > 0 && ctx->sp_ts == nullptr) { void* q = nullptr; if (hipMalloc(&q, (size_t)8192 * 32 * sizeof(long long)) == hipSuccess) { ctx->sp_ts = (long long*)q; ctx->sp_allocs_dbg = q; } }
    if (ctx->sp_ts != nullptr) hipMemset(ctx->sp_ts, 0, (size_t)8192 * 32 * sizeof(long long));
  }
  else if (which == 23) ctx->attn_split = value;
  else if (which == 25) ctx->dbg_trip_group = value;
  else if (which == 26) ctx->sub_serial = value;
  else if (which == 27) ctx->qkv_products = value == 3 ? 3 : 2;
  else if (which == 28) ctx->ffn_compose = value;
  else if (which == 31) ctx->use_lists = value;
  else if (which == 32) ctx->qkv_in_tail = value ? 1 : 0;
  else if (which == 33) ctx->skinny = value;
  else if (which == 48) ctx->prep_fused = value ? 1 : 0;
  else if (which == 29) {
    GN_HIP(hipSetDevice(ctx->device));
    for (int i = 0; i < 8; ++i) if (ctx->sub_s[i]) { hipStreamSynchronize(ctx->sub_s[i]); hipEventDestroy(ctx->ev_join[i]); hipStreamDestroy(ctx->sub_s[i]); ctx->sub_s[i] = nullptr; ctx->ev_join[i] = nullptr; }
    ctx->cu_mask_mode = value;
    if (ctx->n_sub > 1) { const int n = ctx->n_sub; ctx->n_sub = 1; return gn_set_substreams(ctx, n); }
  }
  else return GN_ERR_ARG;
  return GN_OK;
}

int gn_debug_epnp(gn_ctx* ctx, int n, const double* pws, const double* us, double* out, void* stream) {
  if (!ctx || n < 1 || !pws || !us || !out) return GN_ERR_ARG;
  GN_HIP(hipSetDevice(ctx->device));
  launch_epnp_debug(pws, us, out, n, (hipStream_t)stream);
  GN_HIP(hipGetLastError());
  return GN_OK;
}

int gn_debug_lds_dma_probe(gn_ctx* ctx, const float* pattern, unsigned int* out, int blocks, int spin, void* stream) {
  if (!ctx || !pattern || !out || blocks < 1) return GN_ERR_ARG;
  GN_HIP(hipSetDevice(ctx->device));
  launch_lds_dma_probe(pattern, out, blocks, spin, (hipStream_t)stream);
  GN_HIP(hipGetLastError());
  return GN_OK;
}

int gn_debug_mfma_probe(gn_ctx* ctx, int blocks, int iters, void* stream) {
  if (!ctx || blocks < 1 || iters == 0) return GN_ERR_ARG;
  GN_HIP(hipSetDevice(ctx->device));
  launch_mfma_probe(ctx->ls, blocks, iters, (hipStream_t)stream);
  GN_HIP(hipGetLastError());
  return GN_OK;
}

int gn_set_kernel_timing(gn_ctx* ctx, int max_launches) {
  if (!ctx || max_launches < 0) return GN_ERR_ARG;
  hipSetDevice(ctx->device);
  while ((int)ctx->kflops.size() < max_launches) {
    hipEvent_t a, b;
    if (hipEventCreate(&a) != hipSuccess || hipEventCreate(&b) != hipSuccess) return GN_ERR_HIP;
    ctx->kev.push_back(a); ctx->kev.push_back(b); ctx->kflops.push_back(0.0); ctx->kbytes.push_back(0.0); ctx->kclass.push_back(0); ctx->kname.push_back("");
  }
  ctx->ktiming = max_launches > 0;
  ctx->kused = 0;
  return GN_OK;
}

int gn_get_kernel_stats(gn_ctx* ctx, int kernel_class, double* out3) {
  if (!ctx || !out3 || kernel_class < 0 || kernel_class > 1) return GN_ERR_ARG;
  hipSetDevice(ctx->device);
  double ms = 0.0, fl = 0.0, n = 0.0;
  for (size_t i = 0; i < ctx->kused; ++i) {
    if (hipEventSynchronize(ctx->kev[2 * i + 1]) != hipSuccess) return GN_ERR_HIP;
    float t = 0.f;
    if (hipEventElapsedTime(&t, ctx->kev[2 * i], ctx->kev[2 * i + 1]) != hipSuccess) return GN_ERR_HIP;
    if (ctx->kclass[i] != kernel_class) continue;
    ms += t; fl += ctx->kflops[i]; n += 1.0;
  }
  out3[0] = n; out3[1] = ms; out3[2] = fl;
  return GN_OK;
}

int gn_get_kernel_table(gn_ctx* ctx, char* json, int capacity) {
  if (!ctx || !json || capacity < 64) return GN_ERR_ARG;
  hipSetDevice(ctx->device);
  std::map<std::string, std::vector<double>> tab;
  for (size_t i = 0; i < ctx->kused; ++i) {
    if (hipEventSynchronize(ctx->kev[2 * i + 1]) != hipSuccess) return GN_ERR_HIP;
    float t = 0.f;
    if (hipEventElapsedTime(&t, ctx->kev[2 * i], ctx->kev[2 * i + 1]) != hipSuccess) return GN_ERR_HIP;
    std::vector<double>& v = tab[ctx->kname[i] ? ctx->kname[i] : "?"];
    if (v.empty()) v.assign(4, 0.0);
    v[0] += 1.0; v[1] += t; v[2] += ctx->kflops[i]; v[3] += ctx->kbytes[i];
  }
  std::string out = "[";
  bool first = true;
  for (const auto& kv : tab) {
    char buf[512];
    snprintf(buf, sizeof buf, "%s{\"name\": \"%s\", \"launches\": %.0f, \"ms\": %.6f, \"flops\": %.6e, \"bytes\": %.6e}", first ? "" : ", ",
             kv.first.c_str(), kv.second[0], kv.second[1], kv.second[2], kv.second[3]);
    out += buf; first = false;
  }
  out += "]";
  if ((int)out.size() + 1 > capacity) return GN_ERR_ARG;
  memcpy(json, out.c_str(), out.size() + 1);
  return (int)out.size();
}

int gn_get_kernel_bytes(gn_ctx* ctx, int kernel_class, double* out1) {
  if (!ctx || !out1 || kernel_class < 0 || kernel_class > 1) return GN_ERR_ARG;
  double by = 0.0;
  for (size_t i = 0; i < ctx->kused; ++i)
    if (ctx->kclass[i] == kernel_class) by += ctx->kbytes[i];
  *out1 = by;
  return GN_OK;
}

int gn_set_stage_timing(gn_ctx* ctx, int enable) {
  if (!ctx) return GN_ERR_ARG;
  ctx->timing = enable != 0;
  ctx->n_ev = 0;
  return GN_OK;
}

int gn_get_stage_ms(gn_ctx* ctx, float* host_ms, int max_stages) {
  if (!ctx || !host_ms) return GN_ERR_ARG;
  hipSetDevice(ctx->device);
  for (int i = 0; i < ST_COUNT; ++i) ctx->stage_ms[i] = 0.f;
  if (ctx->n_ev > 0) {
    if (hipEventSynchronize(ctx->ev[2 * (ctx->n_ev - 1) + 1]) != hipSuccess) return GN_ERR_HIP;
    for (int i = 0; i < ctx->n_ev; ++i) {
      float ms = 0.f;
      if (hipEventElapsedTime(&ms, ctx->ev[2 * i], ctx->ev[2 * i + 1]) == hipSuccess) ctx->stage_ms[ctx->ev_stage[i]] += ms;
    }
  }
  const int n = max_stages < ST_COUNT ? max_stages : (int)ST_COUNT;
  for (int i = 0; i < n; ++i) host_ms[i] = ctx->stage_ms[i];
  return n;
}

}
```

### gisnav_amd/csrc/gn_attention.hip

```cpp
#include <type_traits>

#include "gn_common.h"

namespace gn {

namespace {
constexpr int KT = 64;
constexpr int KLS = 68;
constexpr int QB = 128;

__global__ __launch_bounds__(256) void k_attn_f32(AttnArgs a) {
  __shared__ __attribute__((aligned(16))) float smem[KT * KLS + KT * 64];
  float* Ks = smem;
  float* Vs = smem + KT * KLS;

  const int tid = threadIdx.x, lane = tid & 63, wave = tid >> 6;
  const int hh = lane >> 5, ql = lane & 31;
  const int h = blockIdx.y, bs = blockIdx.z;
  const int kvs = a.cross ? (bs ^ 1) : bs;
  const int nkv = a.nvalid[kvs];
  const int q0 = blockIdx.x * QB + wave * 32;

  float qf[8][4];
  {
// ... 765 lines not shown
    for (int kt = 0; kt < 2; ++kt)
#pragma unroll
      for (int r = 0; r < 16; ++r) S[kt][r] = 0.f;
#pragma unroll
    for (int c = 0; c < 4; ++c)
#pragma unroll
      for (int kt = 0; kt < 2; ++kt) S[kt] = mfma16<F16>(kf[buf][kt][c], qf[c], S[kt]);
    if (t * KT + KT > nkv) {
#pragma unroll
      for (int kt = 0; kt < 2; ++kt)
#pragma unroll
        for (int r = 0; r < 16; ++r) {
          const int key = t * KT + kt * 32 + (r & 3) + 8 * (r >> 2) + 4 * hh;
          if (key >= nkv) S[kt][r] = -INFINITY;
        }
    }
    float m = fmaxf(S[0][0], S[1][0]);
#pragma unroll
    for (int kt = 0; kt < 2; ++kt)
#pragma unroll
      for (int r = 1; r < 16; r += 2) m = fmaxf(fmaxf(m, S[kt][r]), S[kt][(r + 1) & 15]);
    m = fmaxf(m, __shfl_xor(m, 32));
    if (__builtin_amdgcn_ballot_w64((m - m_run) * kLog2e > 8.0f) != 0) {
      const float m_new = fmaxf(m_run, m);
      const float alpha = __builtin_amdgcn_exp2f((m_run - m_new) * kLog2e);
#pragma unroll
      for (int r = 0; r < 16; ++r) { o[0][r] *= alpha; o[1][r] *= alpha; ol[r] *= alpha; }
      m_run = m_new;
    }
    const float mneg = -m_run * kLog2e;
#pragma unroll
    for (int kt = 0; kt < 2; ++kt)
#pragma unroll
      for (int u = 0; u < 2; ++u) {
        u32x4 pw;
#pragma unroll
        for (int e = 0; e < 4; ++e) {
          const float p0 = __builtin_amdgcn_exp2f(__builtin_fmaf(S[kt][8 * u + 2 * e], kLog2e, mneg));
          const float p1 = __builtin_amdgcn_exp2f(__builtin_fmaf(S[kt][8 * u + 2 * e + 1], kLog2e, mneg));
          pw[e] = pack16<F16>(p0, p1);
        }
        const bf16x8 pf = __builtin_bit_cast(bf16x8, pw);
        ol = mfma16<F16>(ones, pf, ol);
#pragma unroll
        for (int d = 0; d < 2; ++d) o[d] = mfma16<F16>(vf[buf][kt][u][d], pf, o[d]);
      }
  };
#pragma unroll 1
  for (int t0 = wave; t0 < ntiles; t0 += 16) {
#pragma unroll
    for (int i = 0; i < TP; ++i)
      if (t0 + NW * i < ntiles) load_tile(i, t0 + NW * i);
#pragma unroll
    for (int i = 0; i < TP; ++i)
      if (t0 + NW * i < ntiles) tile(i, t0 + NW * i);
  }
#pragma unroll
  for (int d = 0; d < 2; ++d)
#pragma unroll
    for (int r = 0; r < 16; ++r) part[wave][16 * d + r][lane] = o[d][r];
  part[wave][32][lane] = m_run;
  part[wave][33][lane] = ol[0];
  __syncthreads();
  float al[NW], M = -INFINITY, L = 0.f;
#pragma unroll
  for (int i = 0; i < NW; ++i) M = fmaxf(M, part[i][33][lane] > 0.f ? part[i][32][lane] : -INFINITY);
#pragma unroll
  for (int i = 0; i < NW; ++i) {
    const float li = part[i][33][lane];
    al[i] = li > 0.f ? __builtin_amdgcn_exp2f((part[i][32][lane] - M) * kLog2e) : 0.f;
    L += li * al[i];
  }
  const float inv = L > 0.f ? 1.0f / L : 0.f;
  constexpr int GP = 8 / NW;
  float amax = 0.f;
#pragma unroll
  for (int gg = 0; gg < GP; ++gg) {
    const int d = (GP * wave + gg) >> 2, g = (GP * wave + gg) & 3;
    float w4[4];
#pragma unroll
    for (int e = 0; e < 4; ++e) {
      float acc = 0.f;
#pragma unroll
      for (int i = 0; i < NW; ++i) acc += part[i][16 * d + 4 * g + e][lane] * al[i];
      w4[e] = acc * inv;
    }
    const size_t row = (size_t)bs * a.npad + q0 + ql;
    if (a.outp != nullptr) {
      typedef _Float16 f16x4 __attribute__((ext_vector_type(4)));
      typedef float f32x4v __attribute__((ext_vector_type(4)));
      const f32x4v w = {w4[0], w4[1], w4[2], w4[3]};
      ovf_track(amax, w.x, w.y); ovf_track(amax, w.z, w.w);
      const f16x4 hv = __builtin_convertvector(w, f16x4);
      const f16x4 mv = __builtin_convertvector(w - __builtin_convertvector(hv, f32x4v), f16x4);
      uint16_t* pp = a.outp + hm16_off(row, a.ldo, h * 64 + d * 32 + 8 * g + 4 * hh);
      *reinterpret_cast<f16x4*>(pp) = hv;
      *reinterpret_cast<f16x4*>(pp + 16) = mv;
    } else {
      *reinterpret_cast<float4*>(a.out + row * a.ldo + h * 64 + 4 * hh + d * 32 + 8 * g) = make_float4(w4[0], w4[1], w4[2], w4[3]);
    }
  }
  if (a.outp != nullptr) ovf_commit(a.ovf, amax);
}
}

int g_attn_f32_ks = 0;
void launch_attention_f32(const AttnArgs& a, hipStream_t s) {
  if ((g_attn_f32_ks & 3) == 2 || ((g_attn_f32_ks & 3) == 0 && a.BS <= 4)) {
    if (g_attn_f32_ks & 4) hipLaunchKernelGGL(k_attn_f32_ks<8>, dim3(a.npad / 32, kHeads, a.BS), dim3(512), 0, s, a);
    else hipLaunchKernelGGL(k_attn_f32_ks<4>, dim3(a.npad / 32, kHeads, a.BS), dim3(256), 0, s, a);
    g_last_kernel = "k_attn_f32_ks(";
    return;
  }
  dim3 grid(a.npad / QB, kHeads, a.BS), block(256);
  hipLaunchKernelGGL(k_attn_f32, grid, block, 0, s, a);
  g_last_kernel = "k_attn_f32(";
}

void launch_attention_bf16(const AttnArgs& a, hipStream_t s) {
  dim3 grid(a.npad / QB, kHeads, a.BS), block(256);
  hipLaunchKernelGGL(k_attn_bf16, grid, block, 0, s, a);
  g_last_kernel = "k_attn_bf16(";
}

}

namespace gn {
namespace {
__global__ void k_pack_attn_bf16(const float* q, int ldq, const float* k, int ldk, const float* v, int ldv, float qscale,
                                 uint16_t* qb, uint16_t* kb, int ldb, uint16_t* vt, long long ntok, int npad, int f16) {
  const long long idx = (long long)blockIdx.x * blockDim.x + threadIdx.x;
  if (idx >= ntok * 32) return;
  const long long tok = idx >> 5;
  const int g8 = (int)(idx & 31), bs = (int)(tok / npad), i = (int)(tok % npad);
  const int r = i & 15, sp = (i & ~15) + ((r & 3) | ((r & 4) << 1) | ((r & 8) >> 1));
#pragma unroll
  for (int e = 0; e < 8; ++e) {
    const int d = 8 * g8 + e;
    const float qf = q[tok * ldq + d] * qscale, kf = k[tok * ldk + d], vf = v[tok * ldv + d];
    qb[tok * ldb + d] = (unsigned short)(pack16_rt(qf, 0.f, f16) & 0xffffu);
    kb[tok * ldb + d] = (unsigned short)(pack16_rt(kf, 0.f, f16) & 0xffffu);
    vt[(((size_t)bs * kHeads + (d >> 6)) * kHeadDim + (d & 63)) * npad + sp] = (unsigned short)(pack16_rt(vf, 0.f, f16) & 0xffffu);
  }
}
}
void launch_pack_attn_bf16(const AttnArgs& a, uint16_t* qkb, uint16_t* vtb, hipStream_t s) {
  const long long ntok = (long long)a.BS * a.npad;
  hipLaunchKernelGGL(k_pack_attn_bf16, dim3((unsigned)((ntok * 32 + 255) / 256)), dim3(256), 0, s, a.q, a.ldq, a.k, a.ldk, a.v, a.ldv, a.qscale,
                     qkb, qkb + kDim, 2 * kDim, vtb, ntok, a.npad, a.half_fmt);
}
thread_local long long* g_attn_stamps = nullptr;
thread_local int g_attn_variant = 4;
void launch_attention_bf16_v2(const AttnArgs& a, hipStream_t s) {
  const bool pw_auto = g_attn_variant == 4 && a.half_fmt && a.npad % 256 == 0 && (long long)(a.npad / 256) * kHeads * a.BS >= 256;
  if ((pw_auto || g_attn_variant == 70 || g_attn_variant == 73) && !(a.nsplit > 1 && a.part != nullptr) &&
      launch_attention_pw(a, g_attn_variant == 73, s)) return;
  {
    const bool ks_auto = g_attn_variant == 4 && a.BS <= 2;
    if ((ks_auto || g_attn_variant == 80 || g_attn_variant == 81) && !(a.nsplit > 1 && a.part != nullptr) && a.npad % 64 == 0) {
      const dim3 grid(a.npad / 32, kHeads, a.BS);
      if (g_attn_variant == 81) {
        if (a.half_fmt) { hipLaunchKernelGGL((k_attn_ks<true, 4>), grid, dim3(256), 0, s, a); g_last_kernel = "k_attn_ks<true, 4>"; }
        else { hipLaunchKernelGGL((k_attn_ks<false, 4>), grid, dim3(256), 0, s, a); g_last_kernel = "k_attn_ks<false, 4>"; }
      } else {
        if (a.half_fmt) { hipLaunchKernelGGL((k_attn_ks<true, 8>), grid, dim3(512), 0, s, a); g_last_kernel = "k_attn_ks<true, 8>"; }
        else { hipLaunchKernelGGL((k_attn_ks<false, 8>), grid, dim3(512), 0, s, a); g_last_kernel = "k_attn_ks<false, 8>"; }
      }
      return;
    }
  }
  g_last_kernel = "k_attn16_v5<0, 4, 3, 1, false, false>";
  if (a.half_fmt) {
    if (a.nsplit > 1 && a.part != nullptr && a.tickets != nullptr) {
      hipLaunchKernelGGL((k_attn16_v5<0, 4, 3, 1, true, true>), dim3(a.npad / 128 * a.nsplit, kHeads, a.BS), dim3(256), 0, s, a);
      g_last_kernel = "k_attn16_v5<0, 4, 3, 1, true, true>";
      return;
    }
    if (g_attn_variant == 60) { hipLaunchKernelGGL((k_attn16_v5<0, 4, 3, 1, false, true>), dim3(a.npad / 128, kHeads, a.BS), dim3(256), 0, s, a); g_last_kernel = "k_attn16_v5<0, 4, 3, 1, false, true>"; }
    else { hipLaunchKernelGGL((k_attn16_v5<128, 4, 3, 1, false, true>), dim3(a.npad / 128, kHeads, a.BS), dim3(256), 0, s, a); g_last_kernel = "k_attn16_v5<128, 4, 3, 1, false, true>"; }
    return;
  }
  if (a.nsplit > 1 && a.part != nullptr && a.tickets != nullptr && (g_attn_variant == 4 || g_attn_variant == 59)) {
    hipLaunchKernelGGL((k_attn16_v5<0, 4, 3, 1, true>), dim3(a.npad / 128 * a.nsplit, kHeads, a.BS), dim3(256), 0, s, a);
    g_last_kernel = "k_attn16_v5<0, 4, 3, 1, true, false>";
    return;
  }
  dim3 grid(a.npad / 128, kHeads, a.BS), block(256);
  if (g_attn_variant == 56) hipLaunchKernelGGL((k_attn16_v5<128, 4>), grid, block, 0, s, a);
  else hipLaunchKernelGGL((k_attn16_v5<0, 4>), grid, block, 0, s, a);
}
}
```

### gisnav_amd/csrc/gn_attention_pw.hip

```cpp
#include "gn_common.h"
#include <type_traits>

namespace gn {

namespace {
constexpr int KT = 64;
constexpr float kLog2e = 1.4426950408889634f;
constexpr int kRing = 64 * 64;
constexpr int kSlabPitch = 272;
typedef __attribute__((address_space(3))) void* lptr_t;
typedef unsigned int u32x4 __attribute__((ext_vector_type(4)));
#define GN_PIN() __builtin_amdgcn_sched_barrier(0)

template <bool F16> __device__ __forceinline__ f32x16 mfma16(const bf16x8& x, const bf16x8& y, const f32x16& c) {
  if constexpr (F16) {
    typedef _Float16 f16x8_t __attribute__((ext_vector_type(8)));
    return __builtin_amdgcn_mfma_f32_32x32x16_f16(__builtin_bit_cast(f16x8_t, x), __builtin_bit_cast(f16x8_t, y), c, 0, 0, 0);
  } else {
    return __builtin_amdgcn_mfma_f32_32x32x16_bf16(x, y, c, 0, 0, 0);
  }
}
template <bool F16> __device__ __forceinline__ void mfma_v0(f32x16& s, const bf16x8& x, const bf16x8& y) {
  if constexpr (F16) asm volatile("v_mfma_f32_32x32x16_f16 %0, %1, %2, 0" : "=&v"(s) : "v"(x), "v"(y));
  else asm volatile("v_mfma_f32_32x32x16_bf16 %0, %1, %2, 0" : "=&v"(s) : "v"(x), "v"(y));
// ... 91 lines not shown
    return *reinterpret_cast<const bf16x8*>(lds + (stage_byte + kfo[kt][c]));
  };
  auto v_frag = [&](unsigned stage_byte, int d, int kt, int u) __attribute__((always_inline)) {
    return *reinterpret_cast<const bf16x8*>(lds + (stage_byte + vfo[d][kt][u]));
  };

  f32x16 Sa[NQ], Sb[NQ];
  bf16x8 pf[NQ][2];
  float mloc[NQ];
  bool grow = false;

  float mt[NQ][5];
  auto m_step = [&](f32x16 (&S)[NQ], int qi, int st, int key0, auto mask_tag) __attribute__((always_inline)) {
    if (st == 0) {
      if constexpr (decltype(mask_tag)::value) {
        const int lim = nkv - key0 - 4 * hh;
#pragma unroll
        for (int r = 0; r < 16; ++r)
          if ((r & 3) + 8 * (r >> 2) >= lim) S[qi][r] = -INFINITY;
      }
#pragma unroll
      for (int i = 0; i < 5; ++i) mt[qi][i] = __builtin_fmaxf(__builtin_fmaxf(S[qi][3 * i], S[qi][3 * i + 1]), S[qi][3 * i + 2]);
    } else if (st == 1) {
      const float x = __builtin_fmaxf(__builtin_fmaxf(mt[qi][0], mt[qi][1]), mt[qi][2]);
      const float y = __builtin_fmaxf(__builtin_fmaxf(mt[qi][3], mt[qi][4]), S[qi][15]);
      mloc[qi] = __builtin_fmaxf(x, y);
    } else {
      grow = grow || (mloc[qi] - m_run[qi]) * kLog2e > 8.0f;
    }
  };
  auto rescale = [&]() __attribute__((always_inline)) {
    if (__builtin_amdgcn_ballot_w64(grow) != 0) {
#pragma unroll
      for (int qi = 0; qi < NQ; ++qi) {
        const unsigned mu = __float_as_uint(mloc[qi]);
        const auto sw = __builtin_amdgcn_permlane32_swap(mu, mu, false, false);
        const unsigned lo = sw[0], hi = sw[1];
        const float m_new = fmaxf(m_run[qi], __builtin_fmaxf(__uint_as_float(lo), __uint_as_float(hi)));
        const float alpha = __builtin_amdgcn_exp2f((m_run[qi] - m_new) * kLog2e);
#pragma unroll
        for (int r = 0; r < 16; ++r) { o[qi][0][r] *= alpha; o[qi][1][r] *= alpha; ol[qi][r] *= alpha; }
        m_run[qi] = m_new;
      }
    }
    grow = false;
#pragma unroll
    for (int qi = 0; qi < NQ; ++qi) mneg[qi] = -m_run[qi] * kLog2e;
  };
  float xe[8];
  auto e_step = [&](const f32x16 (&S)[NQ], int f, int st) __attribute__((always_inline)) {
    const int qi = f & 1, u = f >> 1;
    if (st < 2) {
#pragma unroll
      for (int e = 4 * st; e < 4 * st + 4; ++e) xe[e] = __builtin_fmaf(S[qi][8 * u + e], kLog2e, mneg[qi]);
    } else if (st < 4) {
#pragma unroll
      for (int e = 4 * (st - 2); e < 4 * (st - 2) + 4; ++e) xe[e] = __builtin_amdgcn_exp2f(xe[e]);
    } else {
      u32x4 pw;
#pragma unroll
      for (int e = 0; e < 4; ++e) pw[e] = pack16<F16>(xe[2 * e], xe[2 * e + 1]);
      pf[qi][u] = __builtin_bit_cast(bf16x8, pw);
    }
  };

  __builtin_amdgcn_s_waitcnt(0);
  asm volatile("s_barrier" ::: "memory");
  stamp(1);

  bf16x8 kf[3];
  if (ntiles > 0) {
#pragma unroll
    for (int c = 0; c < 4; ++c) {
      const bf16x8 kk = k_frag(0, 0, c);
#pragma unroll
      for (int qi = 0; qi < NQ; ++qi) { if (c == 0) mfma_v0<F16>(Sa[qi], kk, qf[qi][c]); else mfma_v<F16>(Sa[qi], kk, qf[qi][c]); }
    }
    asm volatile("s_nop 7\n\ts_nop 7\n\ts_nop 7" : "+v"(Sa[0]), "+v"(Sa[1]));
#pragma unroll
    for (int qi = 0; qi < NQ; ++qi) { m_step(Sa, qi, 0, 0, std::true_type{}); m_step(Sa, qi, 1, 0, std::true_type{}); m_step(Sa, qi, 2, 0, std::true_type{}); }
    rescale();
    kf[0] = k_frag(0, 1, 0);
    kf[1] = k_frag(0, 1, 1);
  }
  stamp(2);

  auto subtile = [&](const f32x16 (&SC)[NQ], f32x16 (&SN)[NQ], unsigned kst, int ktn, unsigned kst2, int kt2, unsigned vst, int kt, int next_key0,
                     auto mask, bool live) __attribute__((always_inline)) {
    bf16x8 vf[2][2];
#pragma unroll
    for (int c = 0; c < 4; ++c) {
#pragma unroll
      for (int qi = 0; qi < NQ; ++qi) {
        const int m = 2 * c + qi;
        if (c == 0) mfma_v0<F16>(SN[qi], kf[c % 3], qf[qi][c]); else mfma_v<F16>(SN[qi], kf[c % 3], qf[qi][c]);
#pragma unroll
        for (int st = (10 * m) / 8; st < (10 * (m + 1)) / 8; ++st) e_step(SC, st / 5, st % 5);
        if (qi == 0) {
          __builtin_amdgcn_sched_barrier(0);
          if (c < 2) kf[(c + 2) % 3] = k_frag(kst, ktn, c + 2);
          vf[c & 1][c >> 1] = v_frag(vst, c & 1, kt, c >> 1);
        }
        GN_PIN();
      }
    }
#pragma unroll
    for (int u = 0; u < 2; ++u) {
#pragma unroll
      for (int i = 0; i < 6; ++i) {
        const int qi = i & 1, m = 6 * u + i;
        if (u == 1 && i == 0) kf[0] = k_frag(kst2, kt2, 0);
        if (u == 1 && i == 2) kf[1] = k_frag(kst2, kt2, 1);
        if (i < 2) ol[qi] = mfma16<F16>(ones, pf[qi][u], ol[qi]);
        else o[qi][(i - 2) >> 1] = mfma16<F16>(vf[(i - 2) >> 1][u], pf[qi][u], o[qi][(i - 2) >> 1]);
        if (m < 6) {
#pragma unroll
          for (int st = (10 * m) / 6; st < (10 * (m + 1)) / 6; ++st) e_step(SC, 2 + st / 5, st % 5);
        } else {
          const int mm = m - 6;
          if (mm < 2) m_step(SN, mm, 0, next_key0, mask);
          else if (mm == 2) { m_step(SN, 0, 1, next_key0, mask); m_step(SN, 1, 1, next_key0, mask); }
          else if (mm == 3) { m_step(SN, 0, 2, next_key0, mask); m_step(SN, 1, 2, next_key0, mask); }
        }
        GN_PIN();
      }
    }
    asm volatile("" ::"v"(SN[0]), "v"(SN[1]));
    if (live) rescale(); else grow = false;
  };

  int k0 = 0, k1 = 1, k2 = 2, k3 = 3;
  int v0 = 0, v1 = 1, v2 = 2;
  auto tile = [&](int t, auto mask_a, auto mask_b) __attribute__((always_inline)) {
    if (t + 2 < ntiles) asm volatile("s_waitcnt vmcnt(4) lgkmcnt(0)\n\ts_barrier" ::: "memory");
    else asm volatile("s_waitcnt vmcnt(0) lgkmcnt(0)\n\ts_barrier" ::: "memory");
    if (t + 3 < ntiles) GN_DMA_K(k3, t + 3);
    if (t + 2 < ntiles) GN_DMA_V(v2, t + 2);
    const unsigned ks0 = 2 * kRing * k0, ks1 = 2 * kRing * k1, vs0 = 2 * kRing * (NDK + v0);
    GN_PIN();
    subtile(Sa, Sb, ks0, 1, ks1, 0, vs0, 0, t * KT + 32, mask_a, true);
    subtile(Sb, Sa, ks1, 0, ks1, 1, vs0, 1, t * KT + 64, mask_b, t + 1 < ntiles);
    { const int s_ = k0; k0 = k1; k1 = k2; k2 = k3; k3 = s_; }
    { const int s_ = v0; v0 = v1; v1 = v2; v2 = s_; }
  };
#pragma unroll 1
  for (int t = 0; t + 2 < ntiles; ++t) tile(t, std::false_type{}, std::false_type{});
  if (ntiles >= 2) tile(ntiles - 2, std::false_type{}, std::true_type{});
  if (ntiles >= 1) tile(ntiles - 1, std::true_type{}, std::false_type{});
  stamp(3);
  stamp(4);
#undef GN_DMA_K
#undef GN_DMA_V

  if (a.outp != nullptr) {
    typedef _Float16 f16x4 __attribute__((ext_vector_type(4)));
    typedef float f32x4v __attribute__((ext_vector_type(4)));
    unsigned char* const slab = reinterpret_cast<unsigned char*>(smem) + 2 * (NDK + NDV) * kRing + wave * 32 * kSlabPitch;
    const int nq = a.nvalid[bs];
    float amax = 0.f;
#pragma unroll
    for (int qi = 0; qi < NQ; ++qi) {
      const float l = ol[qi][0];
      const float inv = l > 0.f ? 1.0f / l : 0.f;
      float amq = 0.f;
#pragma unroll
      for (int d = 0; d < 2; ++d)
#pragma unroll
        for (int g = 0; g < 4; ++g) {
          const f32x4v w = {o[qi][d][4 * g + 0] * inv, o[qi][d][4 * g + 1] * inv, o[qi][d][4 * g + 2] * inv, o[qi][d][4 * g + 3] * inv};
          ovf_track(amq, w.x, w.y); ovf_track(amq, w.z, w.w);
          const f16x4 hv = __builtin_convertvector(w, f16x4);
          const f16x4 mv = __builtin_convertvector(w - __builtin_convertvector(hv, f32x4v), f16x4);
          unsigned char* pp = slab + ql * kSlabPitch + (2 * d + (g >> 1)) * 64 + (8 * (g & 1) + 4 * hh) * 2;
          *reinterpret_cast<f16x4*>(pp) = hv;
          *reinterpret_cast<f16x4*>(pp + 32) = mv;
        }
      if (q0 + 32 * qi + ql < nq) amax = fmaxf(amax, amq);
#pragma unroll
      for (int j = 0; j < 8; ++j) {
        const int row = 4 * j + (lane >> 4), ch = lane & 15;
        const uint4 val = *reinterpret_cast<const uint4*>(slab + row * kSlabPitch + ch * 16);
        uint16_t* dst = a.outp + hm16_off((size_t)bs * a.npad + q0 + 32 * qi + row, a.ldo, h * 64) + ch * 8;
        *reinterpret_cast<uint4*>(dst) = val;
      }
    }
    ovf_commit(a.ovf, amax);
  } else {
#pragma unroll
    for (int qi = 0; qi < NQ; ++qi) {
      const float l = ol[qi][0];
      const float inv = l > 0.f ? 1.0f / l : 0.f;
      float* op = a.out + ((size_t)bs * a.npad + q0 + 32 * qi + ql) * a.ldo + h * 64 + 4 * hh;
#pragma unroll
      for (int d = 0; d < 2; ++d)
#pragma unroll
        for (int g = 0; g < 4; ++g) {
          float4 w;
          w.x = o[qi][d][4 * g + 0] * inv; w.y = o[qi][d][4 * g + 1] * inv;
          w.z = o[qi][d][4 * g + 2] * inv; w.w = o[qi][d][4 * g + 3] * inv;
          *reinterpret_cast<float4*>(op + d * 32 + 8 * g) = w;
        }
    }
  }
  asm volatile("s_waitcnt lgkmcnt(0)\n\ts_barrier" ::: "memory");
  if (ABL & 8) {
    asm volatile("s_waitcnt vmcnt(0)" ::: "memory");
    stamp(5);
    if (lane == 0) {
      long long* dst = reinterpret_cast<long long*>(a.part) + ((size_t)(blockIdx.x + gridDim.x * (blockIdx.y + gridDim.y * blockIdx.z)) * NW + wave) * 8;
      for (int k = 0; k < 6; ++k) dst[k] = ts[k];
      dst[6] = ntiles; dst[7] = 0;
    }
  }
  }
}
#undef GN_PIN
}

bool launch_attention_pw(const AttnArgs& a, bool stamps, hipStream_t s) {
  if (a.npad % 256 != 0 || a.qb == nullptr) return false;
  const int nitems = a.npad / 256 * kHeads * a.BS;
  if (nitems < 8) return false;
  const int ncu = a.ncu >= 8 ? a.ncu : std::max(device_cu_count(), 8);
  const dim3 grid((unsigned)((stamps || nitems < ncu) ? (nitems & ~7) : (ncu & ~7))), block(256);
  if (a.half_fmt) {
    if (stamps) {
      if (g_attn_stamps == nullptr) return false;
      AttnArgs b = a; b.part = reinterpret_cast<float*>(g_attn_stamps); b.tiles = nullptr;
      hipLaunchKernelGGL((k_attn_pw<true, 8>), grid, block, 0, s, b, nitems);
    }
    else hipLaunchKernelGGL((k_attn_pw<true, 0>), grid, block, 0, s, a, nitems);
    g_last_kernel = "k_attn_pw<true, 0>";
  } else {
    hipLaunchKernelGGL((k_attn_pw<false, 0>), grid, block, 0, s, a, nitems);
    g_last_kernel = "k_attn_pw<false, 0>";
  }
  return true;
}

}
```

### gisnav_amd/csrc/gn_common.h

```cpp
#pragma once
#include <hip/hip_runtime.h>
#include <stdint.h>
#include <string>
#include <vector>
#include <map>

#include "../../include/gisnav_amd.h"

namespace gn {

constexpr int kDim = 256;
constexpr int kHeads = 4;
constexpr int kHeadDim = 64;
constexpr int kInDim = 128;
constexpr int kFreq = 32;
constexpr int kMaxLayers = 9;
constexpr int kRecordFloats = 133;

typedef float f32x4 __attribute__((ext_vector_type(4)));
typedef float f32x16 __attribute__((ext_vector_type(16)));
typedef short bf16x8 __attribute__((ext_vector_type(8)));

__device__ __forceinline__ float gelu_erf(float y) {
  const float t = fminf(fabsf(y) * 0.70710678118654752440f, 4.0f);
  float q = 4.6081331674940884e-05f;
  q = q * t + -0.00045161080197431147f;
  q = q * t + 0.0015096671413630247f;
  q = q * t + 0.0007409505778923631f;
  q = q * t + -0.028223754838109016f;
  q = q * t + 0.1484677642583847f;
  q = q * t + 0.918419361114502f;
  q = q * t + 1.6279083490371704f;
  const float e = 1.0f - __builtin_amdgcn_exp2f(-(q * t));
  return 0.5f * y * (1.0f + copysignf(e, y));
}

__host__ __device__ inline size_t hm16_off(size_t row, int ld, int col) {
  return row * (size_t)ld * 2 + (size_t)(col >> 4) * 32 + (col & 15);
}

__device__ __forceinline__ void ovf_track(float& amax, float a, float b) { amax = fmaxf(amax, fmaxf(fabsf(a), fabsf(b))); }
__device__ __forceinline__ void ovf_commit(unsigned int* flag, float amax) { if (flag != nullptr && !(amax < 65504.0f)) atomicOr(flag, 1u); }

template <bool F16> __device__ __forceinline__ unsigned int pack16(float lo, float hi) {
  typedef float f32x2_p __attribute__((ext_vector_type(2)));
  if constexpr (F16) {
    typedef _Float16 f16x2_p __attribute__((ext_vector_type(2)));
    return __builtin_bit_cast(unsigned int, __builtin_convertvector((f32x2_p){lo, hi}, f16x2_p));
  } else {
    typedef __bf16 bf16x2_p __attribute__((ext_vector_type(2)));
    return __builtin_bit_cast(unsigned int, __builtin_convertvector((f32x2_p){lo, hi}, bf16x2_p));
  }
}
__device__ __forceinline__ unsigned int pack16_rt(float lo, float hi, int f16) { return f16 ? pack16<true>(lo, hi) : pack16<false>(lo, hi); }

enum GemmEpi { EPI_BIAS = 0, EPI_SCALE_COLS = 1, EPI_ROTARY = 2, EPI_RESIDUAL = 3, EPI_PLAIN = 4,
               EPI_ROTARY_BF16 = 5, EPI_SCALE_BF16 = 6,
               EPI_LN_GELU = 7,
               EPI_RELU = 8 };

struct GemmArgs {
  const float* A;    int lda;
  const float* A2;   int lda2;
  int K1;
  const float* W;    int ldw;
  const uint16_t* Wp; long long wp_plane;
  float acc_scale;
  const float* bias;
  float* Y;          int ldy;
  int M, N, K;
  long long strideA, strideW, strideY;
  float scale; int scale_cols;
  const float* cos_t; const float* sin_t; int rot_cols;
  const float* resid; int ldr;
  const uint16_t* residp; int ldrp;
  int drop_f32;
  const float* ln_g; const float* ln_b;
  uint16_t* Yb; int ldyb; uint16_t* Vt; int vt_start; int q_cols; float qscale; int npad;
  int vt_perm;
  int half_fmt;
  const uint16_t* Ap;
  const uint16_t* A2p;
  uint16_t* Yp; int ldyp;
  unsigned int* ovf;
  const int* mlim; int mlim_mul; int mlim_seg;
};
void launch_gemm_f32(int epi, const GemmArgs& a, int batch, hipStream_t s);
void launch_gemm_p2(int epi, const GemmArgs& a, int batch, hipStream_t s);
void launch_mfma_probe(float* out, int blocks, int iters, hipStream_t s);
void launch_lds_dma_probe(const float* pattern, unsigned int* out, int blocks, int spin, hipStream_t s);
extern int g_gemm_m64;
extern int g_gemm_r64;
extern int g_attn_f32_ks;
extern int g_lf_conv_knob;
extern thread_local const char* g_last_kernel;
extern thread_local int g_gemm_variant;
extern int g_p2_wide;

struct FfnArgs {
  const uint16_t* xp;
  const uint16_t* mp;
  int composed = 0;
  const uint16_t* cp;
  const uint16_t* wos; float wo_scale; const float* bo;
  const uint16_t* w1s; float w1_scale;
  const float* b1; const float* ln_g; const float* ln_b;
  const uint16_t* w2s; float w2_scale;
  const float* b2;
  uint16_t* yp;
  float* y;
  int T;
  unsigned int* ovf;
  long long* dbg_ts;
  const int* tiles = nullptr;
  int walk = 0;
  const int32_t* nvalid = nullptr; int npad = 0;
  int ncu = 0;
  int products = 3;
  int qkv = 0;
  const uint16_t* q_wf = nullptr; float q_acc_scale = 1.f; const float* q_bias = nullptr;
  const float* q_rot4 = nullptr; long long q_rot_stride = 0;
  uint16_t* q_qkb = nullptr; uint16_t* q_vt = nullptr;
  float q_qscale = 1.f, q_scale = 1.f;
};
void launch_ffn_fused(const FfnArgs& a, hipStream_t s);
bool ffn_selects_128(const FfnArgs& a);
void launch_ffn128(const FfnArgs& a, int stamps, hipStream_t s);
extern int g_ffn_stamps;
extern int g_ffn_shape;
extern int g_sp_conv_h;
void build_weight_fragments(const float* w, int N, int K, float scale, int permute_k, uint16_t* out);

struct QkvArgs {
  const uint16_t* xp;
  const uint16_t* wf; float acc_scale; const float* bias;
  const float* rot4; long long rot_stride;
  uint16_t* qkb; int ldyb;
  uint16_t* vt; int npad;
  float qscale;
  float scale;
  int vt_perm;
  int T;
  int half_fmt;
  unsigned int* ovf;
  long long* dbg_ts;
  const int* tiles = nullptr;
  int products = 2;
  int ncu = 0;
};
void launch_qkv(const QkvArgs& a, bool cross, hipStream_t s);
void launch_skinny_qkv(const QkvArgs& a, bool cross, hipStream_t s);
struct SkinnyTailArgs {
  const uint16_t* xp = nullptr; const uint16_t* cp = nullptr;
  const uint16_t* w1 = nullptr; float w1_scale = 1.f; const float* b1 = nullptr;
  float* h = nullptr;
  const float* ln_g = nullptr; const float* ln_b = nullptr;
  const uint16_t* w2 = nullptr; float w2_scale = 1.f; const float* b2 = nullptr;
  uint16_t* xp_out = nullptr; float* y = nullptr;
  unsigned int* ovf = nullptr; int T = 0;
};
void launch_skinny_h(const SkinnyTailArgs& a, hipStream_t s, int variant = 0);
void launch_skinny_out(const SkinnyTailArgs& a, hipStream_t s, int variant = 0);
int device_cu_count();

struct AttnArgs {
  const uint16_t* qb; int ldqb;
  const uint16_t* kb; int ldkb;
  const uint16_t* vt;
  const float* q; int ldq;
  const float* k; int ldk;
  const float* v; int ldv;
  float* out; int ldo;
  uint16_t* outp;
  const int32_t* nvalid;
  int npad;
  int cross;
  float qscale;
  int BS;
  unsigned int* ovf;
  int half_fmt = 0;
  int nsplit = 1;
  float* part = nullptr;
  unsigned int* tickets = nullptr;
  const int* tiles = nullptr;
  int ncu = 0;
};
constexpr int kTileListBase = 16;
void launch_tile_lists(const int32_t* nvalid, int BS, int npad, int* lists, unsigned long long* feedback , hipStream_t s);
void launch_attention_f32(const AttnArgs& a, hipStream_t s);
void launch_attention_bf16(const AttnArgs& a, hipStream_t s);
void launch_attention_f16x2(const AttnArgs& a, hipStream_t s);
void launch_attention_bf16_v2(const AttnArgs& a, hipStream_t s);
bool launch_attention_pw(const AttnArgs& a, bool stamps, hipStream_t s);
void launch_pack_attn_bf16(const AttnArgs& a, uint16_t* qkb, uint16_t* vtb, hipStream_t s);
extern thread_local long long* g_attn_stamps;
extern thread_local int g_attn_variant;

struct PrepArgs {
  const float* desc_q; const float* kpt_q; const int32_t* n_q; int stride_q;
  const float* desc_r; const float* kpt_r; const int32_t* n_r; int stride_r;
  int kpt_format; int B; int npad;
  const float* wr;
  float* desc;
  float* kxy;
  float* cos_t; float* sin_t;
  int32_t* nvalid;
  float* extent;
  float size_q[2], size_r[2];
  int feature;
  float* x; uint16_t* xp;
  uint16_t* desc_p;
  float* rot4; long long rot_stride;
  unsigned int* ovf_clear; unsigned int ovf_init;
};
void launch_prep(const PrepArgs& a, hipStream_t s);
void launch_ln_gelu(float* h, const float* gamma, const float* beta, int rows, hipStream_t s,
                    uint16_t* hp = nullptr, unsigned int* ovf = nullptr);
void launch_matchability(const float* x, const float* w, const float* b, float* ls, int rows, hipStream_t s);

struct HeadArgs {
  const float* sim;
  const float* ls;
  const int32_t* nvalid;
  int B; int npad; float threshold;
  float* rowmax; float* rowlog; float* colmax; float* collog;
  int32_t* m0; float* max0; int32_t* m1;
  int64_t* idx; float* score; int32_t* n_match; int kmax;
  const unsigned int* ovf;
  const void* md;
  int md_f32;
  float* cpart_m; float* cpart_s; int32_t* cpart_i;
  float* rpart_a; float* rpart_b;
  unsigned int* tickets;
  long long* dbg_ts;
  float* max0b;
  float* rpart_c;
  int32_t* uncert;
  float cert_eps;
  int32_t* uncert_alt = nullptr;
  float cert_eps_alt = -1.f;
  float* colbest = nullptr;
  float* col2 = nullptr;
};
void launch_match_head(const HeadArgs& a, hipStream_t s);
void launch_match_head_fused(const HeadArgs& a, hipStream_t s);

struct GatherArgs {
  const float* kpt_q; int stride_q; const float* kpt_r; int stride_r; int kpt_format;
  const int64_t* idx; const int32_t* n_match; int kmax; int B;
  const uint8_t* dem; int H; int W;
  float* mkp_q; float* obj;
};
void launch_gather(const GatherArgs& a, hipStream_t s);

struct HypResult { double R[9]; double t[3]; int good; int valid; };

struct PnpArgs {
  const float* obj; const float* img; const int32_t* n_pts; int kstride; int B;
  double fx, fy, cx, cy;
  int iterations; float reproj; double confidence; int min_pts;
  double* R; double* t; int32_t* n_inliers; uint8_t* ok;
  uint8_t* mask_ws;
  HypResult* hyp;
  float* pts_ws;
  long long* dbg_ts;
  double sigma_px = 0.0;
  double* cov = nullptr;
  double* sigma_hat = nullptr;
  uint8_t* cov_ok = nullptr;
};
void launch_pnp(const PnpArgs& a, hipStream_t s);
void launch_epnp_debug(const double* pws, const double* us, double* out, int n, hipStream_t s);

struct VoArgs {
  const float* desc_q; const int32_t* n_q; int stride_q;
  const float* desc_r; const int32_t* n_r; int stride_r;
  int B; int npad; double ratio;
  float* desc;
  float* norm2;
  int32_t* nvalid;
  const float* sim;
  int32_t* nn_idx; float* nn_dist;
  uint8_t* good;
  int64_t* idx; float* dist; int32_t* n_good; int kmax;
};
void launch_vo_pack(const VoArgs& a, hipStream_t s);
void launch_vo_knn2(const VoArgs& a, hipStream_t s);

struct WarpArgs {
  const uint8_t* src0; const uint8_t* src1;
  int H, W;
  double M[6];
  int dx, dy, crop_h, crop_w;
  uint8_t* out0; uint8_t* out1;
};
void launch_rotate_crop(const WarpArgs& a, bool fused_gray, hipStream_t s);

constexpr int kSiftMaxOctaves = 12;
struct SiftOctave { float* gauss[6]; float* dog[5]; int w, h; long long stride; };
struct SiftPyramid { SiftOctave oct[kSiftMaxOctaves]; int n_oct; };
struct SiftKeypoint { float x, y, size, angle, response; int octave; };
void sift_gaussian_kernel(double sigma, std::vector<float>& k);
void sift_base_blur(const uint8_t* gray, int B, int h, int w, float* scratch, float* tmp, float* out, long long out_stride, const float* dk, int n, int* counters, hipStream_t s);
void sift_blur(int B, long long stride_in, long long stride_out, const float* in, float* tmp, float* out, int w, int h, const float* dk, int n, hipStream_t s,
               float* dog = nullptr, int in_step = 1, int in_w = 0, float* half_scratch = nullptr);
int sift_tail_first(const SiftPyramid& py, const int* ksize);
void sift_tail(const SiftPyramid& py, int B, int o_first, const float* dk, const int* koff, const int* ksize, hipStream_t s);
void sift_find(const SiftPyramid& py, int B, float threshold, int4* cand, int* counters, int max_cand, hipStream_t s);
void sift_refine(const SiftPyramid& py, int B, const int4* cand, int* counters, int max_cand, SiftKeypoint* kp, long long kp_stride, int max_raw, hipStream_t s);
void sift_descriptors(const SiftPyramid& py, int B, const SiftKeypoint* kp_final, long long kp_stride, const int* counters, int max_n, float* desc, long long out_stride, hipStream_t s);
void sift_sort_dedup(int B, SiftKeypoint* kp, long long kp_stride, int* counters, int max_raw, int max_out,
                     float* kpt_xysa, float* response, int32_t* octave, long long out_stride, hipStream_t s);

void sp_weight_fragments(const float* w, int Cout, int Cin, int taps, int Cout_pad, float* out);
void sp_conv1(const float* in, const float* w, const float* bias, float* out, int B, int H, int W, hipStream_t s, int out_half = 0, unsigned int* ovf = nullptr);
void sp_conv_fused1(const float* gray, const float* w1, const float* b1, int B, int H, int W, const float* bias, float* out, int Cout_pad, hipStream_t s,
                    const uint16_t* wfh, float acc_scale, unsigned int* ovf);
extern int g_sp_fuse1;
extern int g_sp_conv_s, g_sp_nms_fused, g_sp_select_stream;
void sp_weight_fragments_hm16(const float* w, int Cout, int Cin, int taps, int Cout_pad, float scale, uint16_t* out);
void sp_conv(const float* in, int B, int H, int W, int Cin, const float* wf, const float* bias, float* out, int Cout_pad, int taps, int relu, hipStream_t s,
             const uint16_t* wfh = nullptr, float acc_scale = 1.f, unsigned int* ovf = nullptr, int pool = 0,
             int single_product = 0, int in_half = 0, int out_half = 0, long long* dbg_ts = nullptr);
void sp_pool(const float* in, float* out, int B, int H, int W, int C, hipStream_t s);
void sp_scores(const float* logits, int cp, float* scores, int B, int h, int w, hipStream_t s);
void sp_nms(const float* scores, int B, int H, int W, int r, float* pooled, float* tmp, float* mask, float* supp, float* aux, hipStream_t s);
void sp_select(const float* nms, int B, int H, int W, float thr, int border, int* cand, int* counts, int cap, int k,
               float* kpt_xysa, float* score, int* kp_index, long long out_stride, hipStream_t s);
void sp_describe(const float* dmap, int B, int h, int w, const float* kpt_xysa, const int* counts, long long out_stride, int max_k, float* desc, hipStream_t s);

void launch_cast_bf16(const float* in, uint16_t* out, long long n, hipStream_t s);
void launch_split3_bf16(const float* in, uint16_t* planes, long long n, hipStream_t s);
void launch_split2_f16(const float* in, uint16_t* planes, long long n, float scale, hipStream_t s);
void launch_split_hm16(const float* in, uint16_t* out, long long rows, int cols, float scale, hipStream_t s);
void launch_rot_table(const float* cos_t, const float* sin_t, float* rot4, int T, long long stride, hipStream_t s);

}
```

### gisnav_amd/csrc/gn_ffn128.hip

```cpp
#include "gn_common.h"
#include <algorithm>
#include "gn_ffn_util.h"

namespace gn {

namespace {

#define GN_PIN() __builtin_amdgcn_sched_barrier(0)

__device__ __forceinline__ float resid_lo(unsigned int h, float y) { float r; asm("v_fma_mix_f32 %0, %1, -1.0, %2 op_sel:[0,0,0] op_sel_hi:[1,0,0]" : "=v"(r) : "v"(h), "v"(y)); return r; }
__device__ __forceinline__ float addh_lo(unsigned int h, float y) { float r; asm("v_fma_mix_f32 %0, %1, 1.0, %2 op_sel:[0,0,0] op_sel_hi:[1,0,0]" : "=v"(r) : "v"(h), "v"(y)); return r; }
__device__ __forceinline__ float addh_hi(unsigned int h, float y) { float r; asm("v_fma_mix_f32 %0, %1, 1.0, %2 op_sel:[1,0,0] op_sel_hi:[1,0,0]" : "=v"(r) : "v"(h), "v"(y)); return r; }
__device__ __forceinline__ float resid_hi(unsigned int h, float y) { float r; asm("v_fma_mix_f32 %0, %1, -1.0, %2 op_sel:[1,0,0] op_sel_hi:[1,0,0]" : "=v"(r) : "v"(h), "v"(y)); return r; }

template <int ABL, bool COMP, bool LOOP = false, int QKV = 0, int PROD = 3>
__global__ __launch_bounds__(256) void k_ffn128(FfnArgs a_in) {
  static_assert(PROD == 3 || (PROD == 2 && COMP), "two partial products: composed form only");
  constexpr int NJ = 4, NI = 4, NO = 2, NW = 4, TM = 128;
  constexpr int KT = TM * 128;
  constexpr int RING = 8 * KT;
  constexpr int STAT = 8 * KT;
  constexpr int CST = STAT + 4096;
  constexpr int SMEM = 10 * KT;
  __shared__ __attribute__((aligned(1024))) unsigned char smem[SMEM];
  const int n_work = a_in.tiles != nullptr ? a_in.tiles[0] : a_in.T / TM;
#pragma unroll 1
  for (int work = blockIdx.x; work < n_work; work += gridDim.x) {
#if defined(__HIP_DEVICE_COMPILE__)
  typedef __attribute__((address_space(4))) const FfnArgs* karg_t;
  karg_t ap = (karg_t)__builtin_amdgcn_kernarg_segment_ptr();
  if (LOOP) asm volatile("" : "+s"(ap));
  const FfnArgs a = *ap;
#else
  const FfnArgs a = a_in;
#endif
  int tid = threadIdx.x;
  asm volatile("" : "+v"(tid));
  const int lane = tid & 63, wave = __builtin_amdgcn_readfirstlane(tid >> 6);
  const int hh = lane >> 5, ql = lane & 31;
  const int bm = (a.tiles != nullptr ? a.tiles[kTileListBase + work] : work) * TM;
  long long ts[12], ts2[16];
  auto stamp = [&](int k) __attribute__((always_inline)) { if (ABL & 8) ts[k] = (long long)__builtin_amdgcn_s_memtime(); };
  stamp(0);
  if (!LOOP && a.nvalid != nullptr) {
    const int slot = bm / a.npad;
    if (bm - slot * a.npad >= a.nvalid[slot]) {
      if (a.y != nullptr) {
        float4* dst = reinterpret_cast<float4*>(a.y + (size_t)bm * kDim);
        for (int i = tid; i < TM * kDim / 4; i += 256) dst[i] = make_float4(0.f, 0.f, 0.f, 0.f);
      }
      return;
    }
  }
  f32x4 b1q = {0.f, 0.f, 0.f, 0.f};
  if (tid < 128) b1q = *reinterpret_cast<const f32x4*>(a.b1 + 4 * tid);

  const __amdgpu_buffer_rsrc_t crs = __builtin_amdgcn_make_buffer_rsrc(const_cast<uint16_t*>(a.cp) + (size_t)bm * 512, 0, TM * 1024, 0x00020000);
  const __amdgpu_buffer_rsrc_t xrs = __builtin_amdgcn_make_buffer_rsrc(const_cast<uint16_t*>(a.xp) + (size_t)bm * 512, 0, TM * 1024, 0x00020000);
  unsigned int soff[4], sdst[4];
  auto stage_addr = [&]() __attribute__((always_inline)) {
    int t_ = tid;
    asm volatile("" : "+v"(t_));
    const int sr = t_ >> 3, sc = t_ & 7;
#pragma unroll
    for (int q = 0; q < 4; ++q) {
      soff[q] = (unsigned int)((sr + 32 * q) * 1024 + sc * 16);
      sdst[q] = (unsigned int)(RING + (sr + 32 * q) * 128 + ((sc ^ swz(sr + 32 * q)) * 16));
    }
  };
  stage_addr();
  uint4 sa0, sa1, sa2, sa3, sb0, sb1, sb2, sb3;
  auto stv = [&](int set, int q) __attribute__((always_inline)) -> uint4& {
    return set == 0 ? (q == 0 ? sa0 : (q == 1 ? sa1 : (q == 2 ? sa2 : sa3))) : (q == 0 ? sb0 : (q == 1 ? sb1 : (q == 2 ? sb2 : sb3)));
  };
  auto stage_load = [&](int t, int q) __attribute__((always_inline)) {
    stv(t & 1, q) = __builtin_bit_cast(uint4, __builtin_amdgcn_raw_buffer_load_b128((COMP ? t >= 8 : t < 8) ? crs : xrs, soff[q], (t & 7) * 128, 0));
  };
  auto stage_write = [&](int t, int q) __attribute__((always_inline)) {
    *reinterpret_cast<uint4*>(smem + sdst[q] + (t & 1) * KT) = stv(t & 1, q);
  };
  unsigned int bo[3][2][4];
  auto window = [&](int w) __attribute__((always_inline)) {
    int l_ = lane;
    asm volatile("" : "+v"(l_));
    const int q_ = l_ & 31, h_ = l_ >> 5;
#pragma unroll
    for (int jp = 0; jp < 2; ++jp)
#pragma unroll
      for (int c = 0; c < 4; ++c) {
        bo[w][jp][c] = (unsigned int)((32 * jp + q_) * 128 + (((2 * c + h_) ^ swz(32 * jp + q_)) * 16)) + 65536u * w;
        asm volatile("" : "+v"(bo[w][jp][c]));
      }
  };
  window(2);
  f16x8 bq[3][2];
  auto read_b = [&](int g, int tile_off, int ks, int j) __attribute__((always_inline)) {
    const int off = tile_off + (j >> 1) * 8192;
#pragma unroll
    for (int pl = 0; pl < (PROD == 2 ? 1 : 2); ++pl) bq[g % 3][pl] = *reinterpret_cast<const f16x8*>(smem + bo[off >> 16][j & 1][2 * ks + pl] + (off & 65535));
  };
  float amax = 0.f;
  unsigned int pb[2][4];
  const unsigned int lane16 = (unsigned int)lane * 16u;
  auto ldw = [&](const __amdgpu_buffer_rsrc_t& rs, int uoff) __attribute__((always_inline)) {
    return __builtin_bit_cast(f16x8, __builtin_amdgcn_raw_buffer_load_b128(rs, lane16, uoff, 0));
  };

  float gy[8], gt[8], gq[8];
  unsigned int gh[4], gm[4];
  f32x4 c2[2], c3[2];
  float rs[NJ], nmr[NJ];
  const float s1 = a.w1_scale;
  const unsigned int cbase = (unsigned int)(CST + hh * 16 + 32 * NI * wave * 4);
  auto tail_stage = [&](int st, int off, int j, int ksp) __attribute__((always_inline)) {
    if (st == 18) {
#pragma unroll
      for (int e = 0; e < 8; e += 2) { amax = fmaxf(amax, fmaxf(fabsf(gy[e]), fabsf(gy[e + 1]))); gh[e >> 1] = pack16<true>(gy[e], gy[e + 1]); }
    } else if (st == 19) {
      if constexpr (PROD == 3) {
#pragma unroll
        for (int e = 0; e < 8; e += 2) { gt[e] = resid_lo(gh[e >> 1], gy[e]); gt[e + 1] = resid_hi(gh[e >> 1], gy[e + 1]); }
      }
    } else if (st == 20) {
    } else if (st == 21) {
      *reinterpret_cast<uint4*>(smem + pb[j & 1][2 * ksp] + (off + (j >> 1) * 8192)) = make_uint4(gh[0], gh[1], gh[2], gh[3]);
      if constexpr (PROD == 3) {
#pragma unroll
        for (int e = 0; e < 8; e += 2) gm[e >> 1] = pack16<true>(gt[e], gt[e + 1]);
        *reinterpret_cast<uint4*>(smem + pb[j & 1][2 * ksp + 1] + (off + (j >> 1) * 8192)) = make_uint4(gm[0], gm[1], gm[2], gm[3]);
      }
    }
  };

  const __amdgpu_buffer_rsrc_t w1b = __builtin_amdgcn_make_buffer_rsrc(const_cast<uint16_t*>(a.w1s) + (size_t)(NI * wave) * 32 * 2 * 512, 0, NI * 32 * 2 * 1024, 0x00020000);
  constexpr int RA = 4;
  f16x8 fa[RA][NI][2];
  auto load_a = [&](int slot, int n2, int i, int pl) __attribute__((always_inline)) {
    fa[slot][i][pl] = ldw(w1b, ((i * 32 + (COMP ? n2 : ((n2 + 16) & 31))) * 2 + pl) * 1024);
  };
  constexpr int B1OFF = COMP ? 0 : RING + KT;
  if constexpr (COMP) {
#pragma unroll
    for (int q = 0; q < 4; ++q) stage_load(0, q);
#pragma unroll
    for (int q = 0; q < 4; ++q) stage_load(1, q);
#pragma unroll
    for (int q = 0; q < RA; ++q)
#pragma unroll
      for (int i = 0; i < NI; ++i)
#pragma unroll
        for (int pl = 0; pl < 2; ++pl) load_a(q, q, i, pl);
    if (tid < 128) *reinterpret_cast<f32x4*>(smem + B1OFF + 16 * tid) = b1q * (1.0f / s1);
#pragma unroll
    for (int q = 0; q < 4; ++q) stage_write(0, q);
#pragma unroll
    for (int q = 0; q < 4; ++q) stage_load(2, q);
    __syncthreads();
    stamp(1); stamp(2); stamp(3);
  } else {
  const __amdgpu_buffer_rsrc_t wob = __builtin_amdgcn_make_buffer_rsrc(const_cast<uint16_t*>(a.wos) + (size_t)(NO * wave) * 16 * 2 * 512, 0, NO * 16 * 2 * 1024, 0x00020000);
  constexpr int RO = 6;
  f16x8 go[RO][NO][2];
#pragma unroll
  for (int q = 0; q < 4; ++q) stage_load(0, q);
#pragma unroll
  for (int q = 0; q < 4; ++q) stage_load(1, q);
#pragma unroll
  for (int q = 0; q < RO; ++q)
#pragma unroll
    for (int o = 0; o < NO; ++o)
#pragma unroll
      for (int pl = 0; pl < 2; ++pl) go[q][o][pl] = ldw(wob, ((o * 16 + q) * 2 + pl) * 1024);
  f32x16 acc0[NO][NJ];
#pragma unroll
  for (int o = 0; o < NO; ++o)
#pragma unroll
    for (int j = 0; j < NJ; ++j)
#pragma unroll
      for (int r = 0; r < 16; ++r) acc0[o][j][r] = 0.f;
#pragma unroll
  for (int q = 0; q < 4; ++q) stage_write(0, q);
#pragma unroll
  for (int q = 0; q < 4; ++q) stage_load(2, q);
  __syncthreads();
  stamp(1);
  f32x4 bo4[NO][4];
  read_b(0, RING, 0, 0);
  read_b(1, RING, 0, 1);
  GN_PIN();
#pragma unroll
  for (int kk = 0; kk < 16; ++kk) {
    const int s = kk >> 1, ks = kk & 1;
#pragma unroll
    for (int j = 0; j < NJ; ++j) {
      const int g = 4 * kk + j, g2 = g + 2, kk2 = g2 >> 2;
      if (kk2 < 16) read_b(g2, RING + ((kk2 >> 1) & 1) * KT, kk2 & 1, g2 & 3);
#pragma unroll
      for (int p = 0; p < 3; ++p)
#pragma unroll
        for (int o = 0; o < NO; ++o) {
          const int m = 6 * j + 2 * p + o;
          acc0[o][j] = __builtin_amdgcn_mfma_f32_32x32x16_f16(go[kk % RO][o][p == 0 ? 1 : 0], bq[g % 3][p == 1 ? 1 : 0], acc0[o][j], 0, 0, 0);
          if (ks == 0 && m % 6 == 1) stage_write(s + 1, m / 6);
          if (m % 6 == 3 && kk >= 1 && kk + RO - 1 < 16) {
            const int lo = (m / 6) >> 1, lpl = (m / 6) & 1;
            go[(kk - 1) % RO][lo][lpl] = ldw(wob, ((lo * 16 + kk + RO - 1) * 2 + lpl) * 1024);
          }
          if (ks == 0 && m % 6 == 5 && s + 3 <= 8) stage_load(s + 3, m / 6);
          if (kk == 12 && m % 6 == 5)
#pragma unroll
            for (int g4 = 0; g4 < 2; ++g4) {
              const int u = 2 * (m / 6) + g4;
              bo4[u >> 2][u & 3] = *reinterpret_cast<const f32x4*>(a.bo + 32 * (NO * wave + (u >> 2)) + 8 * (u & 3) + 4 * hh);
            }
          GN_PIN();
        }
    }
    __syncthreads();
    GN_PIN();
  }
  stamp(2);

#pragma unroll
  for (int q = 0; q < RA - 2; ++q)
#pragma unroll
    for (int i = 0; i < NI; ++i)
#pragma unroll
      for (int pl = 0; pl < 2; ++pl) load_a(q, q, i, pl);
  if (tid < 128) *reinterpret_cast<f32x4*>(smem + B1OFF + 16 * tid) = b1q * (1.0f / s1);
  window(0);
#pragma unroll
  for (int jp = 0; jp < 2; ++jp)
#pragma unroll
    for (int c = 0; c < 4; ++c) pb[jp][c] = bo[0][jp][c] + (unsigned int)(NO * wave * KT);
#pragma unroll
  for (int o = 0; o < NO; ++o)
#pragma unroll
    for (int j = 0; j < NJ; ++j) {
      f32x2v y[8], t[8];
      unsigned int hw[8], mw[8];
#pragma unroll
      for (int k = 0; k < 8; ++k) y[k] = pair(acc0[o][j], 2 * k) * splat2(a.wo_scale) + (f32x2v){bo4[o][k >> 1][2 * (k & 1)], bo4[o][k >> 1][2 * (k & 1) + 1]};
#pragma unroll
      for (int k = 0; k < 8; ++k) { amax = fmaxf(amax, fmaxf(fabsf(y[k][0]), fabsf(y[k][1]))); hw[k] = __builtin_bit_cast(unsigned int, __builtin_convertvector(y[k], f16x2v)); }
#pragma unroll
      for (int k = 0; k < 8; ++k) t[k] = (f32x2v){resid_lo(hw[k], y[k][0]), resid_hi(hw[k], y[k][1])};
#pragma unroll
      for (int k = 0; k < 8; ++k) mw[k] = __builtin_bit_cast(unsigned int, __builtin_convertvector(t[k], f16x2v));
#pragma unroll
      for (int ksp = 0; ksp < 2; ++ksp) {
        *reinterpret_cast<uint4*>(smem + pb[j & 1][2 * ksp] + (o * KT + (j >> 1) * 8192)) = make_uint4(hw[4 * ksp], hw[4 * ksp + 1], hw[4 * ksp + 2], hw[4 * ksp + 3]);
        *reinterpret_cast<uint4*>(smem + pb[j & 1][2 * ksp + 1] + (o * KT + (j >> 1) * 8192)) = make_uint4(mw[4 * ksp], mw[4 * ksp + 1], mw[4 * ksp + 2], mw[4 * ksp + 3]);
      }
      GN_PIN();
    }
  __syncthreads();
  stamp(3);

  }

  f32x16 acc[NI][NJ];
#pragma unroll
  for (int i = 0; i < NI; ++i) {
    f32x4 bi[4];
#pragma unroll
    for (int g = 0; g < 4; ++g) bi[g] = *reinterpret_cast<const f32x4*>(smem + B1OFF + (32 * (NI * wave + i) + 8 * g + 4 * hh) * 4);
#pragma unroll
    for (int g = 0; g < 4; ++g)
#pragma unroll
      for (int c = 0; c < 4; ++c)
#pragma unroll
        for (int j = 0; j < NJ; ++j) acc[i][j][4 * g + c] = bi[g][c];
    GN_PIN();
  }
  if constexpr (!COMP) {
#pragma unroll
    for (int q = RA - 2; q < RA; ++q)
#pragma unroll
      for (int i = 0; i < NI; ++i)
#pragma unroll
        for (int pl = 0; pl < 2; ++pl) load_a(q, q, i, pl);
  }
  uint4 cst_a;
  read_b(0, COMP ? RING : 0, 0, 0);
  GN_PIN();
  auto gemm1_kstep = [&](int n2) __attribute__((always_inline)) {
    const int n = n2 >> 1, ks = n2 & 1;
#pragma unroll
    for (int j = 0; j < NJ; ++j) {
      const int g = 4 * n2 + j, g1 = g + 1, m2 = g1 >> 2, nn = m2 >> 1;
      if (m2 < 32) read_b(g1, (!COMP && nn < 8) ? nn * KT : RING + (nn & 1) * KT, m2 & 1, g1 & 3);
#pragma unroll
      for (int p = 0; p < 3; ++p)
#pragma unroll
        for (int i = 0; i < NI; ++i) {
          if (PROD == 2 && p == 1) continue;
          const int mj = 4 * p + i;
          acc[i][j] = __builtin_amdgcn_mfma_f32_32x32x16_f16(fa[n2 % RA][i][p == 0 ? 1 : 0], bq[g % 3][p == 1 ? 1 : 0], acc[i][j], 0, 0, 0);
          constexpr int kLa0 = PROD == 3 ? 5 : 1, kLa1 = PROD == 3 ? 10 : 9, kSl = PROD == 3 ? 7 : 3;
          if ((COMP || n >= 8) && ks == 0 && n + 1 < 16 && mj == 2) stage_write(n + 1, j);
          if ((mj == kLa0 || mj == kLa1) && n2 >= 1 && n2 + RA - 1 < 32) {
            const int u = 2 * j + (mj == kLa1 ? 1 : 0);
            load_a((n2 - 1) % RA, n2 + RA - 1, u >> 1, u & 1);
          }
          if (ks == 0 && (COMP || n + 3 >= 9) && n + 3 < 16 && mj == kSl) stage_load(n + 3, j);
          if (n2 == 29 && mj == kSl && j == 0) cst_a = *reinterpret_cast<const uint4*>((tid < 128 ? a.ln_g : a.ln_b - 512) + 4 * tid);
          GN_PIN();
        }
    }
    if (COMP || n >= 8) __syncthreads();
    if (n2 == 15) stamp(10);
    if ((ABL & 128) && ks == 1) ts2[n] = (long long)__builtin_amdgcn_s_memtime();
    GN_PIN();
  };
  if constexpr (COMP) {
#pragma unroll
    for (int n2 = 0; n2 < 32; ++n2) gemm1_kstep(n2);
  } else {
#pragma unroll
    for (int n2 = 0; n2 < 7; ++n2) gemm1_kstep(n2);
    window(1);
#pragma unroll
    for (int n2 = 7; n2 < 11; ++n2) gemm1_kstep(n2);
    stage_addr();
#pragma unroll
    for (int n2 = 11; n2 < 15; ++n2) gemm1_kstep(n2);
    window(2);
#pragma unroll
    for (int n2 = 15; n2 < 32; ++n2) gemm1_kstep(n2);
  }
  stamp(4);

  const __amdgpu_buffer_rsrc_t w2b = __builtin_amdgcn_make_buffer_rsrc(const_cast<uint16_t*>(a.w2s) + (size_t)(NO * wave) * 32 * 2 * 512, 0, NO * 32 * 2 * 1024, 0x00020000);
  constexpr int RG = 5;
  f16x8 ga[RG][NO][2];
  auto load_g = [&](int slot, int c, int o, int pl) __attribute__((always_inline)) {
    const int kstep = 8 * ((c >> 1) & 3) + 2 * (c >> 3) + (c & 1);
    ga[slot][o][pl] = ldw(w2b, ((o * 32 + kstep) * 2 + pl) * 1024);
  };
  *reinterpret_cast<uint4*>(smem + CST + 16 * tid) = cst_a;

  {
    float* const stat = reinterpret_cast<float*>(smem + STAT);
#pragma unroll
    for (int j = 0; j < NJ; ++j) {
      const float K = acc[0][j][0];
      f32x2v sd = splat2(0.f), sq = splat2(0.f);
#pragma unroll
      for (int i = 0; i < NI; ++i) {
#pragma unroll
        for (int r = 0; r < 16; r += 2) {
          const f32x2v d = pair(acc[i][j], r) - splat2(K);
          sd += d;
          sq += d * d;
        }
        GN_PIN();
      }
      const float sdl = sd[0] + sd[1], sql = sq[0] + sq[1];
      const float mu = sdl * (1.0f / 64.0f);
      float mean_a = K + mu, m2_a = sql - sdl * mu;
      const float mean_b = __shfl_xor(mean_a, 32), m2_b = __shfl_xor(m2_a, 32);
      const float dl = mean_a - mean_b;
      m2_a = m2_a + m2_b + 32.0f * dl * dl;
      mean_a = 0.5f * (mean_a + mean_b);
      if (hh == 0) *reinterpret_cast<f32x2v*>(stat + ((wave * TM + 32 * j + ql) * 2)) = (f32x2v){mean_a, m2_a};
    }
    __syncthreads();
#pragma unroll
    for (int j = 0; j < NJ; ++j) {
      f32x2v pw[NW];
#pragma unroll
      for (int w4 = 0; w4 < NW; ++w4) pw[w4] = *reinterpret_cast<const f32x2v*>(stat + ((w4 * TM + 32 * j + ql) * 2));
      const float mean = 0.25f * ((pw[0][0] + pw[1][0]) + (pw[2][0] + pw[3][0]));
      float m2 = (pw[0][1] + pw[1][1]) + (pw[2][1] + pw[3][1]);
#pragma unroll
      for (int w4 = 0; w4 < NW; ++w4) { const float dl = pw[w4][0] - mean; m2 += 128.0f * dl * dl; }
      const float rstd = 1.0f / sqrtf(m2 * (s1 * s1) * (1.0f / 512.0f) + 1e-5f);
      rs[j] = rstd * s1;
      nmr[j] = -(mean * s1) * rstd;
    }
  }
  stamp(5);
#pragma unroll
  for (int q = 0; q < RG; ++q)
#pragma unroll
    for (int o = 0; o < NO; ++o)
#pragma unroll
      for (int pl = 0; pl < 2; ++pl) load_g(q, q, o, pl);

  auto gelu_stage = [&](int st, int q, int j, int ksp) __attribute__((always_inline)) {
    if (st == 0) {
#pragma unroll
      for (int gg = 0; gg < 2; ++gg) {
        const int cof = (32 * q + 8 * (2 * ksp + gg)) * 4;
        c2[gg] = *reinterpret_cast<const f32x4*>(smem + cbase + cof);
        c3[gg] = *reinterpret_cast<const f32x4*>(smem + cbase + cof + 2048);
      }
    } else if (st == 1) {
#pragma unroll
      for (int e = 0; e < 8; ++e) gy[e] = acc[q][j][8 * ksp + e] * rs[j] + nmr[j];
    } else if (st == 2) {
#pragma unroll
      for (int e = 0; e < 8; ++e) gy[e] = gy[e] * c2[e >> 2][e & 3] + c3[e >> 2][e & 3];
    } else if (st == 3) {
#pragma unroll
      for (int e = 0; e < 8; ++e) gt[e] = gy[e] * 0.70710678118654752440f;
    } else if (st == 4) {
#pragma unroll
      for (int e = 0; e < 8; ++e) gt[e] = fminf(fabsf(gt[e]), 4.0f);
    } else if (st == 5) {
#pragma unroll
      for (int e = 0; e < 8; ++e) gq[e] = 4.6081331674940884e-05f * gt[e] + -0.00045161080197431147f;
    } else if (st >= 6 && st <= 11) {
      const float cf = st == 6 ? 0.0015096671413630247f : st == 7 ? 0.0007409505778923631f : st == 8 ? -0.028223754838109016f
                     : st == 9 ? 0.1484677642583847f : st == 10 ? 0.918419361114502f : 1.6279083490371704f;
#pragma unroll
      for (int e = 0; e < 8; ++e) gq[e] = gq[e] * gt[e] + cf;
    } else if (st == 12) {
#pragma unroll
      for (int e = 0; e < 8; ++e) gq[e] = gq[e] * gt[e];
    } else if (st == 13) {
#pragma unroll
      for (int e = 0; e < 8; ++e) gq[e] = __builtin_amdgcn_exp2f(-gq[e]);
    } else if (st == 14) {
#pragma unroll
      for (int e = 0; e < 8; ++e) gq[e] = 1.0f - gq[e];
    } else if (st == 15) {
#pragma unroll
      for (int e = 0; e < 8; ++e) gq[e] = copysignf(gq[e], gy[e]);
    } else if (st == 16) {
#pragma unroll
      for (int e = 0; e < 8; ++e) gt[e] = 0.5f * gy[e];
    } else if (st == 17) {
#pragma unroll
      for (int e = 0; e < 8; ++e) gy[e] = gt[e] * gq[e] + gt[e];
    } else if (st >= 18) {
      tail_stage(st, 0, j, ksp);
    }
  };
  auto set_pb = [&](int q) __attribute__((always_inline)) {
#pragma unroll
    for (int jp = 0; jp < 2; ++jp)
#pragma unroll
      for (int c = 0; c < 4; ++c) pb[jp][c] = bo[q & 1][jp][c] + (unsigned int)(wave * KT);
  };
  window(0);
  window(1);
  auto gelu_tile_pk = [&](int q, int j) __attribute__((always_inline)) {
    f32x4 w4[4], b4[4];
#pragma unroll
    for (int g = 0; g < 4; ++g) {
      w4[g] = *reinterpret_cast<const f32x4*>(smem + cbase + (32 * q + 8 * g) * 4);
      b4[g] = *reinterpret_cast<const f32x4*>(smem + cbase + (32 * q + 8 * g) * 4 + 2048);
    }
    f32x2v y[8], t[8], u[8];
#pragma unroll
    for (int k = 0; k < 8; ++k) y[k] = pair(acc[q][j], 2 * k) * splat2(rs[j]) + splat2(nmr[j]);
#pragma unroll
// ... 392 lines not shown
```

Baseline: 5769.

## Write only high fp16 plane of attention context when tail uses two products

When the fused FFN tail runs in two-product mode, it reads only the high fp16 term of the attention context. In that case the attention kernel writes a compact hi-only context buffer at half the row pitch, and the FFN128 kernel stages from it with new address and stage-load logic that issues fewer loads. This roughly halves the context traffic both when attention writes it and when the tail reads it. The cost is more selection logic across attention and FFN, an abort path if the pairing is wrong, and a host-side conversion in the certification path.

Result: faster. 5953, median of 6 (+3.2%).

```diff
diff --git a/gisnav_amd/csrc/gn_api.hip b/gisnav_amd/csrc/gn_api.hip
--- a/gisnav_amd/csrc/gn_api.hip
+++ b/gisnav_amd/csrc/gn_api.hip
@@ -179,6 +179,7 @@
   hipEvent_t ev_head[8] = {};
   float* o_mkp[2] = {nullptr, nullptr}; float* o_obj[2] = {nullptr, nullptr}; int32_t* o_nmatch[2] = {nullptr, nullptr};
   int prep_fused = 1;
+  int ctx_hi = 1;
   int sift_h = 0, sift_w = 0; std::vector<void*> sift_allocs; SiftPyramid sift_py; float* sift_tmp = nullptr;
   float* sift_dk = nullptr; std::vector<std::vector<float>> sift_kernels; std::vector<int> sift_koff;
   int4* sift_cand = nullptr; int* sift_counts = nullptr; SiftKeypoint* sift_kp = nullptr;
@@ -406,7 +407,7 @@
 
 void timed_attention(gn_ctx* c, const AttnArgs& a, bool bf16v2, hipStream_t s) {
   timed_launch(c, s, 1, 4.0 * a.BS * kHeads * (double)a.npad * a.npad * kHeadDim,
-               (double)a.BS * a.npad * kDim * (a.qb ? 2.0 + 2.0 + 2.0 : 12.0) + (double)a.BS * a.npad * kDim * 4.0,
+               (double)a.BS * a.npad * kDim * (a.qb ? 2.0 + 2.0 + 2.0 : 12.0) + (double)a.BS * a.npad * kDim * (a.out_hi_only ? 2.0 : 4.0),
                nullptr, [&] { if (bf16v2) launch_attention_bf16_v2(a, s); else attention(c, a, s); });
 }
 
@@ -503,9 +504,21 @@
 inline int ffn_level(const gn_ctx* c) { return c->attn_f16 == 2 ? 3 : c->ffn_products == 0 ? (ffn_auto(c) ? c->auto_level : 3) : c->ffn_products; }
 inline float cert_eps_now(const gn_ctx* c) { return ffn_auto(c) ? c->cert_eps_lvl[c->auto_level - 2] : c->cert_eps; }
 
-bool ffn(gn_ctx* c, const Block& blk, int T, hipStream_t s, bool keep_f32, const Block* next = nullptr, bool next_cross = false, int np = 0, int vt_perm = 0) {
-  if (skinny_applies(c, T, np) && !(c->skinny & 8) && c->ffn_fused == 3 && c->ffn_compose && tail_folds_out_proj(c, blk, T) && blk.wfc && blk.b1c && !blk.comp_dirty && blk.ffn3.wfn &&
-      c->h && c->ctx_p && gn::g_ffn_stamps == 0 && gn::g_ffn_shape == 0) {
+bool tail_is_skinny(const gn_ctx* c, const Block& blk, int T, int np) {
+  return skinny_applies(c, T, np) && !(c->skinny & 8) && c->ffn_fused == 3 && c->ffn_compose && tail_folds_out_proj(c, blk, T) && blk.wfc && blk.b1c && !blk.comp_dirty && blk.ffn3.wfn &&
+         c->h && c->ctx_p && gn::g_ffn_stamps == 0 && gn::g_ffn_shape == 0;
+}
+bool tail_is_fused(const gn_ctx* c, const Block& blk, int T) { return c->planes_mode && c->x_planes_only && c->ffn_fused == 3 && blk.ffn0.wf && blk.ffn3.wf && T % 64 == 0; }
+bool tail_is_composed(const gn_ctx* c, const Block& blk, int T) { return tail_folds_out_proj(c, blk, T) && c->ffn_compose && blk.wfc && blk.b1c && !blk.comp_dirty; }
+bool ctx_rows_hi_only(const gn_ctx* c, const Block& blk, int T, int np, const AttnArgs& a, bool bf16v2) {
+  if (!c->ctx_hi || !bf16v2 || a.outp == nullptr || !a.half_fmt || gn::g_attn_variant == 73 || !attention_selects_pw(a)) return false;
+  if (tail_is_skinny(c, blk, T, np) || !tail_is_fused(c, blk, T) || !tail_is_composed(c, blk, T) || ffn_level(c) != 2 || gn::g_ffn_stamps != 0) return false;
+  FfnArgs f; f.cp = c->ctx_p; f.T = T;
+  return ffn_selects_128(f);
+}
+
+bool ffn(gn_ctx* c, const Block& blk, int T, hipStream_t s, bool keep_f32, const Block* next = nullptr, bool next_cross = false, int np = 0, int vt_perm = 0, bool ctx_hi = false) {
+  if (tail_is_skinny(c, blk, T, np)) {
     SkinnyTailArgs a;
     a.xp = c->x_p; a.cp = c->ctx_p; a.w1 = blk.wfc; a.w1_scale = blk.wfc_scale; a.b1 = blk.b1c; a.h = c->h; a.ln_g = blk.ln_g; a.ln_b = blk.ln_b;
     a.w2 = blk.ffn3.wfn; a.w2_scale = blk.ffn3.acc_scale; a.b2 = blk.ffn3.b; a.xp_out = c->x_p; a.y = keep_f32 ? c->x : nullptr;
@@ -514,13 +527,13 @@
     timed_launch(c, s, 0, 2.0 * T * 256.0 * 512.0, 4.0 * T * (512.0 + 256.0 + 256.0) + 4.0 * 256.0 * 512.0, nullptr, [&] { launch_skinny_out(a, s, c->skinny >> 4); });
     return false;
   }
-  if (c->planes_mode && c->x_planes_only && c->ffn_fused == 3 && blk.ffn0.wf && blk.ffn3.wf && T % 64 == 0) {
+  if (tail_is_fused(c, blk, T)) {
     FfnArgs f;
     const bool fold = tail_folds_out_proj(c, blk, T);
     f.cp = fold ? c->ctx_p : nullptr; f.wos = blk.proj_out.wf; f.wo_scale = blk.proj_out.acc_scale; f.bo = blk.proj_out.b;
     f.xp = c->x_p; f.mp = c->msg_p; f.w1s = fold ? blk.ffn0.wf2 : blk.ffn0.wf; f.w1_scale = blk.ffn0.acc_scale; f.b1 = blk.ffn0.b; f.ln_g = blk.ln_g; f.ln_b = blk.ln_b;
     f.w2s = blk.ffn3.wf; f.w2_scale = blk.ffn3.acc_scale; f.b2 = blk.ffn3.b; f.yp = c->x_p; f.y = keep_f32 ? c->x : nullptr; f.T = T;
-    const bool comp = fold && c->ffn_compose && blk.wfc && blk.b1c && !blk.comp_dirty;
+    const bool comp = tail_is_composed(c, blk, T);
     if (comp) { f.composed = 1; f.w1s = blk.wfc; f.w1_scale = blk.wfc_scale; f.b1 = blk.b1c; }
     f.ovf = c->guard ? c->ovf : nullptr;
     f.tiles = (c->use_lists && c->lists && gn::g_ffn_stamps == 0) ? c->lists : nullptr;
@@ -528,6 +541,7 @@
     f.ncu = c->ncu;
     f.composed = comp ? 1 : 0;
     f.products = (comp && ffn_level(c) == 2) ? 2 : 3;
+    f.ctx_hi_only = ctx_hi ? 1 : 0;
     const bool fuse_qkv = next != nullptr && c->qkv_in_tail && !c->fused_proj_off && comp && ffn_selects_128(f) && gn::g_ffn_stamps == 0 && c->attn_f16 && c->qkv_products != 3 && !c->qkv_stamps &&
                           c->precision != GN_PREC_F32 && c->attn_variant >= 1 && qkv_projection_applies(c, *next, T, np, vt_perm) && !(vt_perm & 2);
     if (fuse_qkv) {
@@ -541,6 +555,7 @@
     f.dbg_ts = gn::g_ffn_stamps ? reinterpret_cast<long long*>(c->sim) : nullptr;
     double flops = 2.0 * T * (512.0 * 512.0 + 256.0 * 512.0 + ((fold && !comp) ? 256.0 * 256.0 : 0.0));
     double bytes = 4.0 * T * (256.0 + 256.0 + 256.0 + 256.0) + 4.0 * (512.0 * 512.0 + 256.0 * 512.0);
+    if (ctx_hi) bytes -= 2.0 * T * 256.0;
     if (fuse_qkv) {
       const double N = next_cross ? 2.0 * kDim : 3.0 * kDim;
       flops += 2.0 * T * N * kDim;
@@ -608,6 +623,7 @@
     launch_tile_lists(c->nvalid, BS, np, c->lists, (c->tile_feedback && g >= 0 && g < 8) ? c->tile_feedback + g : nullptr, s);
   }
   bool qkv_done = false;
+  bool ctx_hi = false;
   for (int i = 0; i < c->n_layers; ++i) {
     {
       const Block& blk = c->self_blk[i];
@@ -631,6 +647,8 @@
         a.outp = attn_planes ? c->ctx_p : nullptr; a.ovf = (attn_planes && c->guard) ? c->ovf : nullptr;
         a.qb = c->qkb; a.ldqb = 2 * kDim; a.kb = c->qkb + kDim; a.ldkb = 2 * kDim; a.vt = c->vtb; a.half_fmt = c->attn_f16; a.tiles = (c->use_lists && c->lists) ? c->lists : nullptr; a.ncu = c->ncu;
         if (bf16v2) attn_split(c, a);
+        ctx_hi = ctx_rows_hi_only(c, blk, T, np, a, bf16v2);
+        a.out_hi_only = ctx_hi ? 1 : 0;
         timed_attention(c, a, bf16v2, s);
         if (c->planes_mode && !attn_planes) launch_split_hm16(c->ctx, c->ctx_p, T, kDim, 1.0f, s);
       }
@@ -639,7 +657,7 @@
         GemmArgs g = gemm_args(c->ctx, kDim, blk.proj_out, c->msg, kDim, T);
         gemm(c, EPI_BIAS, g, s);
       }
-      { StageTimer tm(c, s, ST_FFN); qkv_done = ffn(c, blk, T, s, false, bf16v2 ? &c->cross_blk[i] : nullptr, true, np, vt_perm); }
+      { StageTimer tm(c, s, ST_FFN); qkv_done = ffn(c, blk, T, s, false, bf16v2 ? &c->cross_blk[i] : nullptr, true, np, vt_perm, ctx_hi); }
     }
     {
       const Block& blk = c->cross_blk[i];
@@ -664,6 +682,8 @@
         a.outp = attn_planes ? c->ctx_p : nullptr; a.ovf = (attn_planes && c->guard) ? c->ovf : nullptr;
         a.qb = c->qkb; a.ldqb = kDim; a.kb = c->qkb; a.ldkb = kDim; a.vt = c->vtb; a.half_fmt = c->attn_f16; a.tiles = (c->use_lists && c->lists) ? c->lists : nullptr; a.ncu = c->ncu;
         if (bf16v2) attn_split(c, a);
+        ctx_hi = ctx_rows_hi_only(c, blk, T, np, a, bf16v2);
+        a.out_hi_only = ctx_hi ? 1 : 0;
         timed_attention(c, a, bf16v2, s);
         if (c->planes_mode && !attn_planes) launch_split_hm16(c->ctx, c->ctx_p, T, kDim, 1.0f, s);
       }
@@ -672,7 +692,7 @@
         GemmArgs g = gemm_args(c->ctx, kDim, blk.proj_out, c->msg, kDim, T);
         gemm(c, EPI_BIAS, g, s);
       }
-      { StageTimer tm(c, s, ST_FFN); qkv_done = ffn(c, blk, T, s, i == c->n_layers - 1, (bf16v2 && i + 1 < c->n_layers) ? &c->self_blk[i + 1] : nullptr, false, np, vt_perm); }
+      { StageTimer tm(c, s, ST_FFN); qkv_done = ffn(c, blk, T, s, i == c->n_layers - 1, (bf16v2 && i + 1 < c->n_layers) ? &c->self_blk[i + 1] : nullptr, false, np, vt_perm, ctx_hi); }
     }
   }
   {
@@ -803,23 +823,31 @@
     c->ktiming = false; c->stop_after = 0; c->guard = 0; c->npad_run = np;
     const int nblk = c->n_layers > 1 ? 1 : 0;
     const int n_lv = (prod0 == 0 || prod0 == 2) ? 2 : 1;
+    bool rows_hi = false;
     for (int lv = 0; lv < n_lv && applicable; ++lv)
     for (int cross = 0; cross < 2 && applicable; ++cross)
       for (int walk = 0; walk < 2 && applicable; ++walk) {
         c->ffn_products = lv == 0 ? 3 : 2;
         const Block& tail = cross ? c->self_blk[0] : c->cross_blk[0];
+        if (lv == 1 && !rows_hi && c->ctx_hi && !tail_is_skinny(c, tail, T, np) && tail_is_fused(c, tail, T) && tail_is_composed(c, tail, T)) {
+          std::vector<uint16_t> hi(h.size());
+          for (size_t i = 0; i < h.size(); ++i) { const _Float16 v = (_Float16)h[i]; memcpy(&hi[i], &v, 2); }
+          GN_HIP(hipStreamSynchronize(0));
+          GN_HIP(hipMemcpy(c->ctx_p, hi.data(), hi.size() * sizeof(uint16_t), hipMemcpyHostToDevice));
+          rows_hi = true;
+        }
         const Block* next = cross ? &c->cross_blk[0] : &c->self_blk[nblk];
         c->use_lists = walk ? 2 : 3;
         GN_HIP(hipMemcpyAsync(c->x_p, c->msg_p, xbytes, hipMemcpyDeviceToDevice, 0));
         GN_HIP(hipMemsetAsync(c->qkb, 0, qbytes, 0)); GN_HIP(hipMemsetAsync(c->vtb, 0, vbytes, 0));
         c->qkv_in_tail = 1;
-        if (!ffn(c, tail, T, 0, false, next, cross != 0, np, 1)) { applicable = false; break; }
+        if (!ffn(c, tail, T, 0, false, next, cross != 0, np, 1, rows_hi)) { applicable = false; break; }
         GN_HIP(hipMemcpyAsync(keep_q, c->qkb, qbytes, hipMemcpyDeviceToDevice, 0));
         GN_HIP(hipMemcpyAsync(keep_v, c->vtb, vbytes, hipMemcpyDeviceToDevice, 0));
         GN_HIP(hipMemcpyAsync(c->x_p, c->msg_p, xbytes, hipMemcpyDeviceToDevice, 0));
         GN_HIP(hipMemsetAsync(c->qkb, 0, qbytes, 0)); GN_HIP(hipMemsetAsync(c->vtb, 0, vbytes, 0));
         c->qkv_in_tail = 0;
-        ffn(c, tail, T, 0, false, next, cross != 0, np, 1);
+        ffn(c, tail, T, 0, false, next, cross != 0, np, 1, rows_hi);
         if (!qkv_projection(c, *next, cross != 0, T, np, 1, 0)) { applicable = false; break; }
         hipLaunchKernelGGL(k_count_diff, dim3(1024), dim3(256), 0, 0, reinterpret_cast<const uint4*>(keep_q), reinterpret_cast<const uint4*>(c->qkb), (cross ? qbytes / 2 : qbytes) / 16, cnt);
         hipLaunchKernelGGL(k_count_diff, dim3(1024), dim3(256), 0, 0, reinterpret_cast<const uint4*>(keep_v), reinterpret_cast<const uint4*>(c->vtb), vbytes / 16, cnt);
@@ -2392,6 +2420,7 @@
   else if (which == 32) ctx->qkv_in_tail = value ? 1 : 0;
   else if (which == 33) ctx->skinny = value;
   else if (which == 48) ctx->prep_fused = value ? 1 : 0;
+  else if (which == 49) ctx->ctx_hi = value ? 1 : 0;
   else if (which == 29) {
     GN_HIP(hipSetDevice(ctx->device));
     for (int i = 0; i < 8; ++i) if (ctx->sub_s[i]) { hipStreamSynchronize(ctx->sub_s[i]); hipEventDestroy(ctx->ev_join[i]); hipStreamDestroy(ctx->sub_s[i]); ctx->sub_s[i] = nullptr; ctx->ev_join[i] = nullptr; }
diff --git a/gisnav_amd/csrc/gn_attention.hip b/gisnav_amd/csrc/gn_attention.hip
--- a/gisnav_amd/csrc/gn_attention.hip
+++ b/gisnav_amd/csrc/gn_attention.hip
@@ -941,9 +941,11 @@
 thread_local long long* g_attn_stamps = nullptr;
 thread_local int g_attn_variant = 4;
 void launch_attention_bf16_v2(const AttnArgs& a, hipStream_t s) {
-  const bool pw_auto = g_attn_variant == 4 && a.half_fmt && a.npad % 256 == 0 && (long long)(a.npad / 256) * kHeads * a.BS >= 256;
-  if ((pw_auto || g_attn_variant == 70 || g_attn_variant == 73) && !(a.nsplit > 1 && a.part != nullptr) &&
-      launch_attention_pw(a, g_attn_variant == 73, s)) return;
+  if (attention_selects_pw(a) && launch_attention_pw(a, g_attn_variant == 73, s)) return;
+  if (a.out_hi_only) {
+    fprintf(stderr, "[gisnav_amd] launch_attention_bf16_v2: compact context rows were asked for on a launch that k_attn_pw does not take\n");
+    abort();
+  }
   {
     const bool ks_auto = g_attn_variant == 4 && a.BS <= 2;
     if ((ks_auto || g_attn_variant == 80 || g_attn_variant == 81) && !(a.nsplit > 1 && a.part != nullptr) && a.npad % 64 == 0) {
diff --git a/gisnav_amd/csrc/gn_attention_pw.hip b/gisnav_amd/csrc/gn_attention_pw.hip
--- a/gisnav_amd/csrc/gn_attention_pw.hip
+++ b/gisnav_amd/csrc/gn_attention_pw.hip
@@ -267,7 +267,36 @@
 #undef GN_DMA_K
 #undef GN_DMA_V
 
-  if (a.outp != nullptr) {
+  if (a.outp != nullptr && a.out_hi_only) {
+    typedef _Float16 f16x4 __attribute__((ext_vector_type(4)));
+    typedef float f32x4v __attribute__((ext_vector_type(4)));
+    unsigned char* const slab = reinterpret_cast<unsigned char*>(smem) + 2 * (NDK + NDV) * kRing + wave * 32 * kSlabPitch;
+    const int nq = a.nvalid[bs];
+    float amax = 0.f;
+#pragma unroll
+    for (int qi = 0; qi < NQ; ++qi) {
+      const float l = ol[qi][0];
+      const float inv = l > 0.f ? 1.0f / l : 0.f;
+      float amq = 0.f;
+#pragma unroll
+      for (int d = 0; d < 2; ++d)
+#pragma unroll
+        for (int g = 0; g < 4; ++g) {
+          const f32x4v w = {o[qi][d][4 * g + 0] * inv, o[qi][d][4 * g + 1] * inv, o[qi][d][4 * g + 2] * inv, o[qi][d][4 * g + 3] * inv};
+          ovf_track(amq, w.x, w.y); ovf_track(amq, w.z, w.w);
+          *reinterpret_cast<f16x4*>(slab + ql * kSlabPitch + (d * 32 + 8 * g + 4 * hh) * 2) = __builtin_convertvector(w, f16x4);
+        }
+      if (q0 + 32 * qi + ql < nq) amax = fmaxf(amax, amq);
+#pragma unroll
+      for (int j = 0; j < 4; ++j) {
+        const int row = 8 * j + (lane >> 3), ch = lane & 7;
+        const uint4 val = *reinterpret_cast<const uint4*>(slab + row * kSlabPitch + ch * 16);
+        uint16_t* dst = a.outp + ((size_t)bs * a.npad + q0 + 32 * qi + row) * a.ldo + h * 64 + ch * 8;
+        *reinterpret_cast<uint4*>(dst) = val;
+      }
+    }
+    ovf_commit(a.ovf, amax);
+  } else if (a.outp != nullptr) {
     typedef _Float16 f16x4 __attribute__((ext_vector_type(4)));
     typedef float f32x4v __attribute__((ext_vector_type(4)));
     unsigned char* const slab = reinterpret_cast<unsigned char*>(smem) + 2 * (NDK + NDV) * kRing + wave * 32 * kSlabPitch;
@@ -332,15 +361,23 @@
 #undef GN_PIN
 }
 
+static bool attention_pw_applies(const AttnArgs& a, bool stamps) {
+  if (a.npad % 256 != 0 || a.qb == nullptr || a.npad / 256 * kHeads * a.BS < 8) return false;
+  if (stamps && a.half_fmt && g_attn_stamps == nullptr) return false;
+  return !a.out_hi_only || (!stamps && a.half_fmt && a.outp != nullptr);
+}
+bool attention_selects_pw(const AttnArgs& a) {
+  const bool pw_auto = g_attn_variant == 4 && a.half_fmt && a.npad % 256 == 0 && (long long)(a.npad / 256) * kHeads * a.BS >= 256;
+  return (pw_auto || g_attn_variant == 70 || g_attn_variant == 73) && !(a.nsplit > 1 && a.part != nullptr) && attention_pw_applies(a, g_attn_variant == 73);
+}
+
 bool launch_attention_pw(const AttnArgs& a, bool stamps, hipStream_t s) {
-  if (a.npad % 256 != 0 || a.qb == nullptr) return false;
+  if (!attention_pw_applies(a, stamps)) return false;
   const int nitems = a.npad / 256 * kHeads * a.BS;
-  if (nitems < 8) return false;
   const int ncu = a.ncu >= 8 ? a.ncu : std::max(device_cu_count(), 8);
   const dim3 grid((unsigned)((stamps || nitems < ncu) ? (nitems & ~7) : (ncu & ~7))), block(256);
   if (a.half_fmt) {
     if (stamps) {
-      if (g_attn_stamps == nullptr) return false;
       AttnArgs b = a; b.part = reinterpret_cast<float*>(g_attn_stamps); b.tiles = nullptr;
       hipLaunchKernelGGL((k_attn_pw<true, 8>), grid, block, 0, s, b, nitems);
     }
diff --git a/gisnav_amd/csrc/gn_common.h b/gisnav_amd/csrc/gn_common.h
--- a/gisnav_amd/csrc/gn_common.h
+++ b/gisnav_amd/csrc/gn_common.h
@@ -117,6 +117,7 @@
   const int32_t* nvalid = nullptr; int npad = 0;
   int ncu = 0;
   int products = 3;
+  int ctx_hi_only = 0;
   int qkv = 0;
   const uint16_t* q_wf = nullptr; float q_acc_scale = 1.f; const float* q_bias = nullptr;
   const float* q_rot4 = nullptr; long long q_rot_stride = 0;
@@ -184,6 +185,7 @@
   unsigned int* tickets = nullptr;
   const int* tiles = nullptr;
   int ncu = 0;
+  int out_hi_only = 0;
 };
 constexpr int kTileListBase = 16;
 void launch_tile_lists(const int32_t* nvalid, int BS, int npad, int* lists, unsigned long long* feedback , hipStream_t s);
@@ -191,6 +193,7 @@
 void launch_attention_bf16(const AttnArgs& a, hipStream_t s);
 void launch_attention_f16x2(const AttnArgs& a, hipStream_t s);
 void launch_attention_bf16_v2(const AttnArgs& a, hipStream_t s);
+bool attention_selects_pw(const AttnArgs& a);
 bool launch_attention_pw(const AttnArgs& a, bool stamps, hipStream_t s);
 void launch_pack_attn_bf16(const AttnArgs& a, uint16_t* qkb, uint16_t* vtb, hipStream_t s);
 extern thread_local long long* g_attn_stamps;
diff --git a/gisnav_amd/csrc/gn_ffn128.hip b/gisnav_amd/csrc/gn_ffn128.hip
--- a/gisnav_amd/csrc/gn_ffn128.hip
+++ b/gisnav_amd/csrc/gn_ffn128.hip
@@ -55,17 +55,31 @@
   f32x4 b1q = {0.f, 0.f, 0.f, 0.f};
   if (tid < 128) b1q = *reinterpret_cast<const f32x4*>(a.b1 + 4 * tid);
 
-  const __amdgpu_buffer_rsrc_t crs = __builtin_amdgcn_make_buffer_rsrc(const_cast<uint16_t*>(a.cp) + (size_t)bm * 512, 0, TM * 1024, 0x00020000);
+  constexpr int NP = PROD == 2 ? 2 : 4;
+  const bool chi = PROD == 2 && a.ctx_hi_only != 0;
+  const int cstep = chi ? 64 : 128;
+  const __amdgpu_buffer_rsrc_t crs = __builtin_amdgcn_make_buffer_rsrc(const_cast<uint16_t*>(a.cp) + (size_t)bm * (chi ? 256 : 512), 0, chi ? TM * 512 : TM * 1024, 0x00020000);
   const __amdgpu_buffer_rsrc_t xrs = __builtin_amdgcn_make_buffer_rsrc(const_cast<uint16_t*>(a.xp) + (size_t)bm * 512, 0, TM * 1024, 0x00020000);
-  unsigned int soff[4], sdst[4];
+  unsigned int soff[4], sdst[4], coff[2];
   auto stage_addr = [&]() __attribute__((always_inline)) {
     int t_ = tid;
     asm volatile("" : "+v"(t_));
-    const int sr = t_ >> 3, sc = t_ & 7;
-#pragma unroll
-    for (int q = 0; q < 4; ++q) {
-      soff[q] = (unsigned int)((sr + 32 * q) * 1024 + sc * 16);
-      sdst[q] = (unsigned int)(RING + (sr + 32 * q) * 128 + ((sc ^ swz(sr + 32 * q)) * 16));
+    if constexpr (PROD == 2) {
+      const int u = t_ >> 2, pc = t_ & 3, sc = 4 * (pc >> 1) + (pc & 1);
+      const int sr = (u & ~3) | ((u & 1) << 1) | ((u >> 1) & 1);
+#pragma unroll
+      for (int q = 0; q < 2; ++q) {
+        soff[q] = (unsigned int)((sr + 64 * q) * 1024 + sc * 16);
+        coff[q] = chi ? (unsigned int)((sr + 64 * q) * 512 + pc * 16) : soff[q];
+        sdst[q] = (unsigned int)(RING + (sr + 64 * q) * 128 + ((sc ^ swz(sr + 64 * q)) * 16));
+      }
+    } else {
+      const int sr = t_ >> 3, sc = t_ & 7;
+#pragma unroll
+      for (int q = 0; q < 4; ++q) {
+        soff[q] = (unsigned int)((sr + 32 * q) * 1024 + sc * 16);
+        sdst[q] = (unsigned int)(RING + (sr + 32 * q) * 128 + ((sc ^ swz(sr + 32 * q)) * 16));
+      }
     }
   };
   stage_addr();
@@ -74,7 +88,12 @@
     return set == 0 ? (q == 0 ? sa0 : (q == 1 ? sa1 : (q == 2 ? sa2 : sa3))) : (q == 0 ? sb0 : (q == 1 ? sb1 : (q == 2 ? sb2 : sb3)));
   };
   auto stage_load = [&](int t, int q) __attribute__((always_inline)) {
-    stv(t & 1, q) = __builtin_bit_cast(uint4, __builtin_amdgcn_raw_buffer_load_b128((COMP ? t >= 8 : t < 8) ? crs : xrs, soff[q], (t & 7) * 128, 0));
+    if constexpr (PROD == 2) {
+      if (t >= 8) stv(t & 1, q) = __builtin_bit_cast(uint4, __builtin_amdgcn_raw_buffer_load_b128(crs, coff[q], (t & 7) * cstep, 0));
+      else stv(t & 1, q) = __builtin_bit_cast(uint4, __builtin_amdgcn_raw_buffer_load_b128(xrs, soff[q], (t & 7) * 128, 0));
+    } else {
+      stv(t & 1, q) = __builtin_bit_cast(uint4, __builtin_amdgcn_raw_buffer_load_b128((COMP ? t >= 8 : t < 8) ? crs : xrs, soff[q], (t & 7) * 128, 0));
+    }
   };
   auto stage_write = [&](int t, int q) __attribute__((always_inline)) {
     *reinterpret_cast<uint4*>(smem + sdst[q] + (t & 1) * KT) = stv(t & 1, q);
@@ -141,9 +160,9 @@
   constexpr int B1OFF = COMP ? 0 : RING + KT;
   if constexpr (COMP) {
 #pragma unroll
-    for (int q = 0; q < 4; ++q) stage_load(0, q);
-#pragma unroll
-    for (int q = 0; q < 4; ++q) stage_load(1, q);
+    for (int q = 0; q < NP; ++q) stage_load(0, q);
+#pragma unroll
+    for (int q = 0; q < NP; ++q) stage_load(1, q);
 #pragma unroll
     for (int q = 0; q < RA; ++q)
 #pragma unroll
@@ -152,9 +171,9 @@
         for (int pl = 0; pl < 2; ++pl) load_a(q, q, i, pl);
     if (tid < 128) *reinterpret_cast<f32x4*>(smem + B1OFF + 16 * tid) = b1q * (1.0f / s1);
 #pragma unroll
-    for (int q = 0; q < 4; ++q) stage_write(0, q);
-#pragma unroll
-    for (int q = 0; q < 4; ++q) stage_load(2, q);
+    for (int q = 0; q < NP; ++q) stage_write(0, q);
+#pragma unroll
+    for (int q = 0; q < NP; ++q) stage_load(2, q);
     __syncthreads();
     stamp(1); stamp(2); stamp(3);
   } else {
@@ -298,12 +317,12 @@
           const int mj = 4 * p + i;
           acc[i][j] = __builtin_amdgcn_mfma_f32_32x32x16_f16(fa[n2 % RA][i][p == 0 ? 1 : 0], bq[g % 3][p == 1 ? 1 : 0], acc[i][j], 0, 0, 0);
           constexpr int kLa0 = PROD == 3 ? 5 : 1, kLa1 = PROD == 3 ? 10 : 9, kSl = PROD == 3 ? 7 : 3;
-          if ((COMP || n >= 8) && ks == 0 && n + 1 < 16 && mj == 2) stage_write(n + 1, j);
+          if ((COMP || n >= 8) && ks == 0 && n + 1 < 16 && mj == 2 && (NP == 4 || j % 2 == 0)) stage_write(n + 1, NP == 4 ? j : j / 2);
           if ((mj == kLa0 || mj == kLa1) && n2 >= 1 && n2 + RA - 1 < 32) {
             const int u = 2 * j + (mj == kLa1 ? 1 : 0);
             load_a((n2 - 1) % RA, n2 + RA - 1, u >> 1, u & 1);
           }
-          if (ks == 0 && (COMP || n + 3 >= 9) && n + 3 < 16 && mj == kSl) stage_load(n + 3, j);
+          if (ks == 0 && (COMP || n + 3 >= 9) && n + 3 < 16 && mj == kSl && (NP == 4 || j % 2 == 0)) stage_load(n + 3, NP == 4 ? j : j / 2);
           if (n2 == 29 && mj == kSl && j == 0) cst_a = *reinterpret_cast<const uint4*>((tid < 128 ? a.ln_g : a.ln_b - 512) + 4 * tid);
           GN_PIN();
         }
```
